# virtuoso/clap

Measured on AMD Instinct MI355X. Metric: entity updates/sec (transform hierarchy + inverse + AABB + frustum cull + visible list), higher is better.
Workload: dtype f32; 1 GPU; BASELINE configs[1]: 1000000 entities/GPU, 125000 chains x depth 8, tiles SoA layout, all dirty, fused frustum cull + ordered visible list (303309 visible); entities_per_gpu=1000000, levels=8, particles_per_gpu=0, exchange=none

## Files before the change

clap_amd/_lib.py:

```python
import ctypes as C
import os
import subprocess

_HERE = os.path.dirname(os.path.abspath(__file__))
LIB_PATH = os.environ.get("CLAPGPU_LIB") or os.path.join(_HERE, "lib", "libclapgpu.so")
CSRC = os.path.join(_HERE, "csrc")
ABI_VERSION = 46

OK = 0
ERR_NOMEM = -1
ERR_INVALID_ARGUMENTS = -2
ERR_NOT_SUPPORTED = -3
ERR_TOO_LARGE = -11
ERR_INIT_FAILED = -14
ERR_OUT_OF_BOUNDS = -26
ERR_UNKNOWN = -32

E_VISIBLE = 1 << 0
E_SKIP_CULLING = 1 << 14
E_DIRTY = 1 << 16
E_JOINT_ATTACHED = 1 << 17
E_ALIVE = 1 << 31
RAY_INVALID = 1 << 0
RAY_UNRESOLVED = 1 << 1
RAY_MOVED_TARGET = 1 << 2
SLIDE_INVALID = 1 << 0
SLIDE_UNRESOLVED = 1 << 1
SLIDE_MOVED_TARGET = 1 << 2
UPDATE_ALL_DIRTY = 1 << 0

_ERR_NAMES = {ERR_NOMEM: "NOMEM", ERR_INVALID_ARGUMENTS: "INVALID_ARGUMENTS", ERR_NOT_SUPPORTED: "NOT_SUPPORTED",
              ERR_TOO_LARGE: "TOO_LARGE", ERR_INIT_FAILED: "INITIALIZATION_FAILED",
              ERR_OUT_OF_BOUNDS: "OUT_OF_BOUNDS", ERR_UNKNOWN: "UNKNOWN_ERROR"}


class ClapGpuError(RuntimeError):
    def __init__(self, code, where, detail=""):
        self.code = code
        super().__init__(f"{where}: CERR_{_ERR_NAMES.get(code, code)} ({code}) {detail}".rstrip())


class Frustum(C.Structure):
    _fields_ = [("planes", C.c_float * 24), ("corners", C.c_float * 32)]


class BvQuery(C.Structure):
    _fields_ = [("cam_pos", C.c_float * 3), ("has_ctl", C.c_uint32), ("ctl_pos", C.c_float * 3),
                ("ctl_entity", C.c_uint32), ("result", C.c_void_p), ("inside_mask", C.c_void_p)]


EXTRA_VIEWS_MAX = 4


class Views(C.Structure):
    _fields_ = [("n", C.c_uint32), ("pad", C.c_uint32), ("frustum", Frustum * EXTRA_VIEWS_MAX),
                ("vis_mask", C.c_void_p * EXTRA_VIEWS_MAX), ("vis_row_pop", C.c_void_p * EXTRA_VIEWS_MAX),
                ("host_vis_mask", C.c_void_p * EXTRA_VIEWS_MAX)]


class Entities(C.Structure):
    _fields_ = [("n", C.c_uint32), ("n_models", C.c_uint32),
                ("pos_scale", C.c_void_p), ("rot", C.c_void_p), ("parent", C.c_void_p),
                ("model", C.c_void_p), ("model_table", C.c_void_p), ("flags", C.c_void_p),
                ("seqs", C.c_void_p), ("mx", C.c_void_p), ("inv_mx", C.c_void_p),
                ("aabb", C.c_void_p), ("center", C.c_void_p), ("vis_mask", C.c_void_p),
                ("vis_row_pop", C.c_void_p), ("n_attach", C.c_uint32), ("pad", C.c_uint32),
                ("attach", C.c_void_p), ("jt_pool", C.c_void_p), ("bind_pool", C.c_void_p),
                ("attach_local", C.c_void_p), ("bv", C.POINTER(BvQuery)), ("rebuilt_mask", C.c_void_p),
                ("views", C.POINTER(Views))]


class Particles(C.Structure):
    _fields_ = [("n", C.c_uint32), ("n_sys", C.c_uint32), ("sys", C.c_void_p), ("row_sys", C.c_void_p),
                ("pos", C.c_void_p), ("vel", C.c_void_p), ("rng_state", C.c_void_p),
                ("billboard_mx", C.c_void_p), ("respawn_mask", C.c_void_p), ("respawn_row_pop", C.c_void_p),
                ("respawn_list", C.c_void_p), ("respawn_count", C.c_void_p), ("scratch", C.c_void_p),
                ("respawn_groups", C.c_void_p)]


class AnimClock(C.Structure):
    _fields_ = [("n_chars", C.c_uint32), ("n_anims", C.c_uint32), ("anim", C.c_void_p), ("time_end", C.c_void_p),
                ("ani_time", C.c_void_p), ("speed", C.c_void_p), ("restart", C.c_void_p), ("frame_time", C.c_void_p),
                ("ended", C.c_void_p)]


class Skeleton(C.Structure):
    _fields_ = [("nr_joints", C.c_uint32), ("n_levels", C.c_uint32), ("parent", C.c_void_p), ("depth", C.c_void_p),
                ("root_pose", C.c_void_p), ("invmx", C.c_void_p), ("bind", C.c_void_p)]


class Animations(C.Structure):
    _fields_ = [("n_anims", C.c_uint32), ("n_times", C.c_uint32), ("chan_table", C.c_void_p),
                ("times", C.c_void_p), ("data", C.c_void_p), ("packed", C.c_void_p), ("packed_keys", C.c_uint32),
                ("packed_layout", C.c_uint32), ("n_data", C.c_uint32), ("pad", C.c_uint32)]


class PoseBatch(C.Structure):
    _fields_ = [("n_chars", C.c_uint32), ("skip", C.c_uint32), ("anim", C.c_void_p), ("frame_time", C.c_void_p), ("entity", C.c_void_p),
                ("entity_mx", C.c_void_p), ("trs", C.c_void_p), ("joint_transforms", C.c_void_p),
                ("joint_pos", C.c_void_p)]


class SkinBatch(C.Structure):
    _fields_ = [("n_chars", C.c_uint32), ("nr_joints", C.c_uint32), ("vert_first", C.c_void_p),
                ("vert_count", C.c_void_p), ("out_first", C.c_void_p), ("position", C.c_void_p),
                ("normal", C.c_void_p), ("joints", C.c_void_p), ("weights", C.c_void_p),
                ("joint_transforms", C.c_void_p), ("out_position", C.c_void_p), ("out_normal", C.c_void_p),
                ("out_w", C.c_void_p)]


class World(C.Structure):
    _fields_ = [("gravity", C.c_double * 3), ("linear_damping", C.c_double),
                ("linear_damping_threshold_sq", C.c_double), ("adis_linear_threshold_sq", C.c_double),
                ("adis_angular_threshold_sq", C.c_double), ("adis_time", C.c_double),
                ("adis_steps", C.c_int32), ("pad", C.c_int32)]


class Bodies(C.Structure):
    _fields_ = [("n", C.c_uint32), ("adis_average_samples", C.c_uint32), ("pos", C.c_void_p), ("quat", C.c_void_p),
                ("lvel", C.c_void_p), ("avel", C.c_void_p), ("mass", C.c_void_p), ("radius", C.c_void_p),
                ("yoffset", C.c_void_p), ("bflags", C.c_void_p), ("adis_steps_left", C.c_void_p),
                ("adis_time_left", C.c_void_p), ("body_entity", C.c_void_p),
                ("length", C.c_void_p), ("inertia", C.c_void_p), ("geom_offset_R", C.c_double * 12),
                ("aabb", C.c_void_p), ("axis", C.c_void_p), ("adis_samples", C.c_void_p), ("adis_counter", C.c_void_p),
                ("geom_records", C.c_void_p), ("facc", C.c_void_p)]


class Geoms(C.Structure):
    _fields_ = [("n", C.c_uint32), ("pad", C.c_uint32), ("pos", C.c_void_p), ("axis", C.c_void_p),
                ("radius", C.c_void_p), ("length", C.c_void_p), ("kind", C.c_void_p), ("aabb", C.c_void_p),
                ("material", C.c_void_p), ("records", C.c_void_p)]


class TrimeshDesc(C.Structure):
    _fields_ = [("n_meshes", C.c_uint32), ("n_statics", C.c_uint32), ("static_index", C.c_void_p), ("vx_first", C.c_void_p),
                ("tri_first", C.c_void_p), ("vx", C.c_void_p), ("idx", C.c_void_p), ("scale", C.c_void_p),
                ("pos", C.c_void_p), ("quat", C.c_void_p)]


POSE_SKIP_TRS, POSE_SKIP_JOINT_POS, POSE_JOINT_POS_MODEL = 1, 2, 4
BODY_DISABLED, BODY_AUTO_DISABLE, BODY_NO_GRAVITY, BODY_GYROSCOPIC, BODY_HAS_JOINT, BODY_KINEMATIC = 1, 2, 4, 8, 16, 32
GEOM_SPHERE, GEOM_CAPSULE, GEOM_BOX, GEOM_OTHER = 0, 1, 2, 3
CONTACT_DEEP = 0x80000000


def mesh_contact_scratch(static_capacity):
    return (int(static_capacity) + 63) // 64 + 1


def bodies_push_scratch_bytes(n):
    return int(lib().clapgpu_bodies_push_scratch_bytes(int(n)))


def bodies_islands_scratch_bytes(n):
    return int(lib().clapgpu_bodies_islands_scratch_bytes(int(n)))


def bodies_solve_scratch_bytes(n, rows_capacity):
    return int(lib().clapgpu_bodies_solve_scratch_bytes(int(n), int(rows_capacity)))


class Slide(C.Structure):
    _fields_ = [("n", C.c_uint32), ("body", C.c_void_p), ("velocity", C.c_void_p), ("airborne", C.c_void_p),
                ("first_frac", C.c_void_p), ("push_hit", C.c_void_p), ("flags", C.c_void_p)]


class CharactersMove(C.Structure):
    _fields_ = [("n", C.c_uint32), ("body", C.c_void_p), ("ray_off", C.c_void_p), ("motion", C.c_void_p),
                ("state", C.c_void_p), ("jump", C.c_void_p), ("jump_params", C.c_void_p), ("velocity", C.c_void_p),
                ("normal", C.c_void_p), ("airborne", C.c_void_p), ("request", C.c_void_p), ("applied", C.c_void_p),
                ("collision", C.c_void_p), ("first_frac", C.c_void_p), ("push_hit", C.c_void_p), ("flags", C.c_void_p),
                ("entity", C.c_void_p), ("yaw_quat", C.c_void_p)]


CS_START, CS_WAKING, CS_IDLE, CS_MOVING, CS_JUMP_START, CS_JUMPING, CS_FALLING, CS_NONE = 0, 1, 2, 3, 4, 5, 6, 0xff


ANIQ_MAX = 4
ANI_END_NONE, ANI_END_IDLE, ANI_END_START_MOTION, ANI_END_ANY_TO_JUMP, ANI_END_HOST = 0, 1, 2, 3, 0xff
(ANI_IDLE, ANI_START_TO_IDLE, ANI_MOTION_STOP, ANI_JUMP_TO_IDLE, ANI_FALL_TO_IDLE, ANI_MOTION, ANI_MOTION_START,
 ANI_JUMP_TO_MOTION, ANI_IDLE_TO_JUMP, ANI_MOTION_TO_JUMP, ANI_JUMP, ANI_FALL, ANI_NAMES) = range(13)
ANI_NAME_LIST = ("idle", "start_to_idle", "motion_stop", "jump_to_idle", "fall_to_idle", "motion", "motion_start",
                 "jump_to_motion", "idle_to_jump", "motion_to_jump", "jump", "fall")
ANIQ_ENDED, ANIQ_STARTED, ANIQ_ADVANCED, ANIQ_CB_IDLE, ANIQ_CB_START_MOTION, ANIQ_CB_ANY_TO_JUMP, ANIQ_HOST, ANIQ_OVERFLOW = (
    1, 2, 4, 8, 16, 32, 64, 128)
ANIQ_STATE_SHIFT = 8


class AniqEntry(C.Structure):
    _fields_ = [("animation", C.c_uint16), ("repeat", C.c_uint8), ("end", C.c_uint8), ("speed", C.c_float)]


class Aniq(C.Structure):
    _fields_ = [("n", C.c_uint32), ("n_anims", C.c_uint32), ("name_anim", C.c_void_p), ("time_end", C.c_void_p),
                ("queue", C.c_void_p), ("len", C.c_void_p), ("cur", C.c_void_p), ("cleared", C.c_void_p),
                ("ani_time", C.c_void_p), ("state", C.c_void_p), ("airborne", C.c_void_p), ("velocity", C.c_void_p),
                ("ch_motion", C.c_void_p), ("jump_params", C.c_void_p), ("mover", C.c_void_p), ("pose_anim", C.c_void_p),
                ("frame_time", C.c_void_p), ("events", C.c_void_p)]


def characters_move_scratch_bytes(n_bodies, n):
    return int(lib().clapgpu_characters_move_scratch_bytes(int(n_bodies), int(n)))


def characters_order_scratch_bytes(n, pair_capacity):
    return int(lib().clapgpu_characters_order_scratch_bytes(int(n), int(pair_capacity)))


def characters_move_ordered_scratch_bytes(n_bodies, n, pair_capacity):
    return int(lib().clapgpu_characters_move_ordered_scratch_bytes(int(n_bodies), int(n), int(pair_capacity)))


class Characters(C.Structure):
    _fields_ = [("n", C.c_uint32), ("limbo_height", C.c_float), ("entity", C.c_void_p), ("body", C.c_void_p),
                ("hist_pos", C.c_void_p), ("hist_head", C.c_void_p), ("hist_wrapped", C.c_void_p),
                ("airborne", C.c_void_p), ("moved", C.c_void_p)]


class Lights(C.Structure):
    _fields_ = [("nr_lights", C.c_uint32), ("pad", C.c_uint32), ("pos", C.c_void_p), ("color", C.c_void_p),
                ("attenuation", C.c_void_p), ("is_dir", C.c_void_p), ("active", C.c_void_p)]


class Solver(C.Structure):
    _fields_ = [("iterations", C.c_uint32), ("wide_rows", C.c_uint32), ("sor_w", C.c_double), ("cfm", C.c_double)]


class FrameDesc(C.Structure):
    _fields_ = [("entities", C.POINTER(Entities)), ("tile_row_start", C.c_void_p), ("n_tiles", C.c_uint32),
                ("level_start", C.c_void_p), ("n_levels", C.c_uint32), ("frustum", C.POINTER(Frustum)),
                ("bodies", C.POINTER(Bodies)), ("world", C.POINTER(World)), ("bp", C.c_void_p),
                ("pairs", C.c_void_p), ("pair_capacity", C.c_uint32), ("pair_total", C.c_void_p),
                ("static_pairs", C.c_void_p), ("static_pair_capacity", C.c_uint32), ("static_pair_total", C.c_void_p),
                ("body_geoms", C.POINTER(Geoms)), ("static_geoms", C.POINTER(Geoms)),
                ("contacts", C.c_void_p), ("static_contacts", C.c_void_p),
                ("contact_total", C.c_void_p), ("static_contact_total", C.c_void_p),
                ("n_body_links", C.c_uint32), ("link_body", C.c_void_p), ("link_entity", C.c_void_p),
                ("characters", C.POINTER(Characters)),
                ("lights", C.POINTER(Lights)),
                ("n_light_carriers", C.c_uint32), ("carrier_entity", C.c_void_p), ("carrier_light", C.c_void_p),
                ("carrier_offset", C.c_void_p),
                ("light_width", C.c_uint32), ("light_height", C.c_uint32), ("light_cell", C.c_uint32), ("light_tiles", C.c_void_p),
                ("view_mx", C.POINTER(C.c_float)), ("proj_mx", C.POINTER(C.c_float)),
                ("anim_clock", C.POINTER(AnimClock)), ("now_dev", C.c_void_p),
                ("skeleton", C.POINTER(Skeleton)), ("animations", C.POINTER(Animations)), ("pose", C.POINTER(PoseBatch)),
                ("skin", C.POINTER(SkinBatch)),
                ("particles", C.POINTER(Particles)),
                ("index_base", C.c_uint32), ("visible", C.c_void_p), ("visible_count", C.c_void_p), ("visible_scratch", C.c_void_p),
                ("cam_pos", C.c_float * 3), ("force_lod", C.c_void_p), ("cur_lod", C.c_void_p), ("draw_lod", C.c_void_p),
                ("flags", C.c_uint32),
                ("meshes", C.c_void_p), ("mesh_contacts", C.c_void_p), ("mesh_ref", C.c_void_p),
                ("mesh_contact_capacity", C.c_uint32), ("mesh_contact_total", C.c_void_p), ("mesh_capped", C.c_void_p),
                ("mesh_scratch", C.c_void_p),
                ("island_scratch", C.c_void_p), ("island", C.c_void_p), ("island_woken", C.c_void_p),
                ("solver", C.POINTER(Solver)), ("solve_scratch", C.c_void_p), ("solve_rows_capacity", C.c_uint32),
                ("solve_status", C.c_void_p),
                ("move", C.POINTER(CharactersMove)), ("move_dt_sec", C.c_double), ("move_scratch", C.c_void_p),
                ("aniq", C.POINTER(Aniq))]


LIGHTS_MAX = 128

STRUCTS = {
    "clapgpu_frustum": Frustum, "clapgpu_bv_query": BvQuery, "clapgpu_views": Views, "clapgpu_entities": Entities,
    "clapgpu_particles": Particles, "clapgpu_anim_clock": AnimClock, "clapgpu_skeleton": Skeleton,
    "clapgpu_animations": Animations, "clapgpu_pose_batch": PoseBatch, "clapgpu_skin_batch": SkinBatch,
    "clapgpu_world": World, "clapgpu_bodies": Bodies, "clapgpu_geoms": Geoms, "clapgpu_trimesh_desc": TrimeshDesc,
    "clapgpu_slide": Slide, "clapgpu_move": CharactersMove, "clapgpu_characters": Characters, "clapgpu_lights": Lights,
    "clapgpu_solver": Solver, "clapgpu_aniq_entry": AniqEntry, "clapgpu_aniq": Aniq, "clapgpu_frame": FrameDesc,
}


SYMBOLS = {
    "clapgpu_device_count": (C.c_int, []),
    "clapgpu_init": (C.c_int, [C.c_int]),
    "clapgpu_last_error": (C.c_char_p, []),
    "clapgpu_test_fail_after": (None, [C.c_int]),
    "clapgpu_abi_version": (C.c_uint32, []),
    "clapgpu_malloc": (C.c_int, [C.POINTER(C.c_void_p), C.c_size_t]),
    "clapgpu_free": (C.c_int, [C.c_void_p]),
    "clapgpu_host_malloc": (C.c_int, [C.POINTER(C.c_void_p), C.c_size_t]),
    "clapgpu_host_free": (C.c_int, [C.c_void_p]),
    "clapgpu_memcpy_h2d": (C.c_int, [C.c_void_p, C.c_void_p, C.c_size_t, C.c_void_p]),
    "clapgpu_memcpy_d2h": (C.c_int, [C.c_void_p, C.c_void_p, C.c_size_t, C.c_void_p]),
    "clapgpu_memset": (C.c_int, [C.c_void_p, C.c_int, C.c_size_t, C.c_void_p]),
    "clapgpu_stream_sync": (C.c_int, [C.c_void_p]),
    "clapgpu_view_matrix": (None, [C.POINTER(C.c_float), C.POINTER(C.c_float), C.POINTER(C.c_float)]),
    "clapgpu_perspective": (None, [C.c_float, C.c_float, C.c_float, C.c_float, C.c_int, C.POINTER(C.c_float)]),
    "clapgpu_frustum_calc": (None, [C.POINTER(C.c_float), C.POINTER(C.c_float), C.c_int, C.POINTER(Frustum)]),
    "clapgpu_entities_update": (C.c_int, [C.c_void_p, C.POINTER(Entities), C.POINTER(C.c_uint32), C.c_uint32,
                                          C.c_uint32, C.POINTER(Frustum)]),
    "clapgpu_entities_update_level": (C.c_int, [C.c_void_p, C.POINTER(Entities), C.c_uint32, C.c_uint32,
                                                C.c_uint32, C.POINTER(Frustum)]),
    "clapgpu_entities_update_tiles": (C.c_int, [C.c_void_p, C.POINTER(Entities), C.c_void_p, C.c_uint32,
                                                C.c_uint32, C.POINTER(Frustum)]),
    "clapgpu_entities_lod": (C.c_int, [C.c_void_p, C.POINTER(Entities), C.c_void_p, C.c_void_p, C.c_uint32,
                                       C.POINTER(C.c_float), C.c_void_p, C.c_void_p, C.c_void_p]),
    "clapgpu_entities_cull": (C.c_int, [C.c_void_p, C.POINTER(Entities), C.POINTER(Frustum)]),
    "clapgpu_visible_scratch_bytes": (C.c_size_t, [C.c_uint32]),
    "clapgpu_visible_compact": (C.c_int, [C.c_void_p, C.c_void_p, C.c_void_p, C.c_uint32, C.c_uint32, C.c_void_p,
                                          C.c_void_p, C.c_void_p]),
    "clapgpu_animation_time": (C.c_int, [C.c_void_p, C.POINTER(AnimClock), C.c_double]),
    "clapgpu_animation_time_dev": (C.c_int, [C.c_void_p, C.POINTER(AnimClock), C.c_void_p]),
    "clapgpu_animations_packed_bytes": (C.c_size_t, [C.c_uint32, C.c_uint32, C.c_uint32]),
    "clapgpu_animations_pack": (C.c_int, [C.c_void_p, C.POINTER(Animations), C.c_uint32, C.c_uint32, C.c_void_p, C.POINTER(C.c_uint32)]),
    "clapgpu_joint_pos_world": (C.c_int, [C.c_void_p, C.POINTER(Skeleton), C.POINTER(PoseBatch)]),
    "clapgpu_pose_update": (C.c_int, [C.c_void_p, C.POINTER(Skeleton), C.POINTER(Animations), C.POINTER(PoseBatch)]),
    "clapgpu_skin": (C.c_int, [C.c_void_p, C.POINTER(SkinBatch)]),
    "clapgpu_phys_step_schedule": (C.c_int, [C.POINTER(C.c_double), C.c_double]),
    "clapgpu_world_defaults": (None, [C.POINTER(World)]),
    "clapgpu_bodies_step": (C.c_int, [C.c_void_p, C.POINTER(Bodies), C.POINTER(World), C.c_double]),
    "clapgpu_phys_body_update": (C.c_int, [C.c_void_p, C.POINTER(Bodies), C.c_uint32, C.c_void_p, C.c_void_p, C.c_void_p,
                                           C.c_void_p]),
    "clapgpu_geom_offset_rotation": (None, [C.POINTER(C.c_double)]),
    "clapgpu_mass_sphere_total": (None, [C.c_double, C.c_double, C.POINTER(C.c_double)]),
    "clapgpu_mass_capsule_total": (None, [C.c_double, C.c_int, C.c_double, C.c_double, C.POINTER(C.c_double)]),
    "clapgpu_capsule_geom": (None, [C.c_float, C.c_float, C.c_float, C.c_double, C.c_double, C.POINTER(C.c_float),
                                    C.POINTER(C.c_float), C.POINTER(C.c_float), C.POINTER(C.c_int), C.POINTER(C.c_float)]),
    "clapgpu_bodies_aabb": (C.c_int, [C.c_void_p, C.POINTER(Bodies)]),
    "clapgpu_bp_create": (C.c_int, [C.POINTER(C.c_void_p), C.c_uint32, C.c_double, C.c_uint32, C.c_void_p]),
    "clapgpu_bp_create_levels": (C.c_int, [C.POINTER(C.c_void_p), C.c_uint32, C.c_double, C.c_uint32, C.c_uint32, C.c_void_p]),
    "clapgpu_bp_levels": (C.c_uint32, [C.c_void_p]),
    "clapgpu_bp_cell_slot": (C.c_uint32, [C.c_void_p, C.c_uint32, C.c_int32, C.c_int32, C.c_int32]),
    "clapgpu_bp_destroy": (None, [C.c_void_p]),
    "clapgpu_bp_collide": (C.c_int, [C.c_void_p, C.c_void_p, C.c_uint32, C.c_void_p, C.c_void_p, C.c_uint32, C.c_void_p,
                                     C.c_void_p, C.c_uint32, C.c_void_p]),
    "clapgpu_bp_status": (C.c_int, [C.c_void_p, C.c_void_p, C.POINTER(C.c_uint32)]),
    "clapgpu_bp_static_aabb": (C.c_void_p, [C.c_void_p]),
    "clapgpu_bp_statics_update": (C.c_int, [C.c_void_p, C.c_void_p, C.c_uint32, C.c_void_p]),
    "clapgpu_bp_statics_sizes": (C.c_int, [C.c_void_p, C.POINTER(C.c_uint32), C.POINTER(C.c_uint32), C.POINTER(C.c_uint32),
                                           C.POINTER(C.c_uint32), C.POINTER(C.c_double)]),
    "clapgpu_bp_statics_read": (C.c_int, [C.c_void_p, C.c_void_p, C.c_void_p, C.c_void_p, C.c_void_p, C.c_void_p, C.c_void_p]),
    "clapgpu_contacts_geoms": (C.c_int, [C.c_void_p, C.POINTER(Geoms), C.POINTER(Geoms), C.c_void_p, C.c_void_p, C.c_uint32,
                                         C.c_void_p, C.c_void_p, C.c_void_p, C.c_void_p]),
    "clapgpu_contacts_geoms_both": (C.c_int, [C.c_void_p, C.c_void_p, C.POINTER(Geoms), C.POINTER(Geoms), C.c_void_p, C.c_void_p,
                                              C.c_uint32, C.c_void_p, C.c_void_p, C.c_void_p, C.c_void_p, C.c_uint32, C.c_void_p,
                                              C.c_void_p, C.c_void_p]),
    "clapgpu_sweep_capsules": (C.c_int, [C.c_void_p, C.POINTER(Geoms), C.POINTER(Geoms), C.c_void_p, C.c_uint32, C.c_void_p,
                                         C.c_void_p, C.c_void_p, C.c_void_p, C.c_void_p, C.c_void_p, C.c_void_p]),
    "clapgpu_bodies_rotate_from_entities": (C.c_int, [C.c_void_p, C.POINTER(Bodies), C.POINTER(Entities), C.c_uint32,
                                                      C.c_uint32, C.c_void_p, C.c_void_p]),
    "clapgpu_contacts_spheres": (C.c_int, [C.c_void_p, C.POINTER(Bodies), C.c_void_p, C.c_void_p, C.c_uint32,
                                           C.c_void_p, C.c_void_p, C.c_void_p]),
    "clapgpu_contacts_sphere_box": (C.c_int, [C.c_void_p, C.POINTER(Bodies), C.c_uint32, C.c_void_p, C.c_void_p,
                                              C.c_void_p, C.c_uint32, C.c_void_p, C.c_void_p, C.c_void_p, C.c_void_p]),
    "clapgpu_shard_tile_range": (C.c_int, [C.c_void_p, C.c_uint32, C.c_uint32, C.c_uint32, C.POINTER(C.c_uint32),
                                           C.POINTER(C.c_uint32)]),
    "clapgpu_bodies_step_prebin": (C.c_int, [C.c_void_p, C.POINTER(Bodies), C.POINTER(World), C.c_double, C.c_void_p]),
    "clapgpu_bp_invalidate": (C.c_int, [C.c_void_p, C.c_void_p]),
    "clapgpu_bp_index": (C.c_int, [C.c_void_p, C.c_void_p, C.c_uint32, C.c_void_p]),
    "clapgpu_bp_index_status": (C.c_int, [C.c_void_p, C.c_void_p, C.POINTER(C.c_uint32)]),
    "clapgpu_bp_leveled_index": (C.c_int, [C.c_void_p, C.c_int]),
    "clapgpu_ray_cast": (C.c_int, [C.c_void_p, C.c_void_p, C.POINTER(Geoms), C.POINTER(Geoms), C.c_void_p, C.c_uint32,
                                   C.c_void_p, C.c_void_p, C.c_void_p, C.c_void_p, C.c_void_p, C.c_void_p]),
    "clapgpu_bodies_ground_collide": (C.c_int, [C.c_void_p, C.c_void_p, C.POINTER(Bodies), C.POINTER(Geoms), C.c_void_p,
                                                C.c_uint32, C.c_void_p, C.c_void_p, C.c_void_p, C.c_void_p, C.c_void_p,
                                                C.c_void_p, C.c_void_p, C.c_void_p, C.c_void_p]),
    "clapgpu_trimesh_create": (C.c_int, [C.c_void_p, C.POINTER(C.c_void_p), C.POINTER(TrimeshDesc)]),
    "clapgpu_trimesh_pose": (C.c_int, [C.c_void_p, C.c_void_p, C.c_void_p, C.c_void_p]),
    "clapgpu_trimesh_status": (C.c_int, [C.c_void_p, C.c_void_p, C.POINTER(C.c_uint32), C.POINTER(C.c_uint32)]),
    "clapgpu_trimesh_destroy": (None, [C.c_void_p]),
    "clapgpu_contacts_meshes": (C.c_int, [C.c_void_p, C.POINTER(Geoms), C.POINTER(Geoms), C.c_void_p, C.c_void_p, C.c_void_p,
                                          C.c_uint32, C.c_void_p, C.c_uint32, C.c_void_p, C.c_void_p, C.c_void_p, C.c_void_p,
                                          C.c_void_p]),
    "clapgpu_sweep_capsules_grid": (C.c_int, [C.c_void_p, C.c_void_p, C.POINTER(Bodies), C.POINTER(Geoms), C.c_void_p, C.c_uint32,
                                              C.c_void_p, C.c_void_p, C.c_void_p, C.c_void_p, C.c_void_p, C.c_void_p]),
    "clapgpu_characters_slide": (C.c_int, [C.c_void_p, C.c_void_p, C.POINTER(Bodies), C.POINTER(Geoms), C.c_void_p, C.c_double,
                                           C.POINTER(Slide), C.c_void_p]),
    "clapgpu_bodies_push_scratch_bytes": (C.c_size_t, [C.c_uint32]),
    "clapgpu_bodies_push": (C.c_int, [C.c_void_p, C.POINTER(Bodies), C.POINTER(World), C.c_uint32, C.c_void_p, C.c_void_p,
                                      C.c_void_p, C.c_void_p, C.c_void_p, C.c_void_p]),
    "clapgpu_characters_move_scratch_bytes": (C.c_size_t, [C.c_uint32, C.c_uint32]),
    "clapgpu_characters_move": (C.c_int, [C.c_void_p, C.c_void_p, C.POINTER(Bodies), C.POINTER(World), C.POINTER(Geoms),
                                          C.c_void_p, C.POINTER(Entities), C.c_double, C.POINTER(CharactersMove), C.c_void_p]),
    "clapgpu_characters_state": (C.c_int, [C.c_void_p, C.POINTER(Aniq), C.POINTER(CharactersMove), C.c_double, C.c_void_p]),
    "clapgpu_animation_queue_time": (C.c_int, [C.c_void_p, C.POINTER(Aniq), C.c_double, C.c_void_p]),
    "clapgpu_characters_order_scratch_bytes": (C.c_size_t, [C.c_uint32, C.c_uint32]),
    "clapgpu_characters_order": (C.c_int, [C.c_void_p, C.c_void_p, C.POINTER(Bodies), C.POINTER(World), C.c_double,
                                           C.POINTER(CharactersMove), C.c_uint32, C.c_void_p, C.c_void_p,
                                           C.POINTER(C.c_uint32), C.c_void_p]),
    "clapgpu_characters_move_ordered_scratch_bytes": (C.c_size_t, [C.c_uint32, C.c_uint32, C.c_uint32]),
    "clapgpu_characters_move_ordered": (C.c_int, [C.c_void_p, C.c_void_p, C.c_void_p, C.POINTER(Bodies), C.POINTER(World),
                                                  C.POINTER(Geoms), C.c_void_p, C.POINTER(Entities), C.c_double,
                                                  C.POINTER(CharactersMove), C.c_uint32, C.c_void_p, C.POINTER(C.c_uint32),
                                                  C.c_void_p]),
    "clapgpu_bodies_islands_scratch_bytes": (C.c_size_t, [C.c_uint32]),
    "clapgpu_bodies_islands": (C.c_int, [C.c_void_p, C.POINTER(Bodies), C.POINTER(World), C.c_double, C.c_void_p, C.c_void_p,
                                         C.c_uint32, C.c_void_p, C.c_void_p, C.c_void_p, C.c_void_p]),
    "clapgpu_solver_defaults": (None, [C.POINTER(Solver)]),
    "clapgpu_bodies_solve_scratch_bytes": (C.c_size_t, [C.c_uint32, C.c_uint32]),
    "clapgpu_bodies_solve": (C.c_int, [C.c_void_p, C.POINTER(Bodies), C.POINTER(World), C.POINTER(Solver), C.c_double, C.c_void_p,
                                       C.c_void_p, C.c_void_p, C.c_uint32, C.c_void_p,
                                       C.c_void_p, C.c_void_p, C.c_void_p, C.c_uint32,
                                       C.c_void_p, C.c_void_p, C.c_uint32, C.c_void_p,
                                       C.c_uint32, C.c_void_p, C.c_void_p, C.c_void_p, C.c_void_p, C.c_void_p,
                                       C.c_void_p, C.c_void_p]),
    "clapgpu_visible_compact_lod": (C.c_int, [C.c_void_p, C.c_void_p, C.c_uint32, C.c_void_p, C.c_void_p, C.c_void_p, C.c_void_p,
                                              C.c_void_p, C.c_void_p, C.c_void_p]),
    "clapgpu_characters_update_clock": (C.c_int, [C.c_void_p, C.c_void_p, C.c_void_p, C.c_void_p, C.c_void_p, C.c_double, C.c_void_p]),
    "clapgpu_host_malloc_mapped": (C.c_int, [C.POINTER(C.c_void_p), C.POINTER(C.c_void_p), C.c_size_t]),
    "clapgpu_entities_apply_inputs": (C.c_int, [C.c_void_p, C.c_void_p, C.c_void_p, C.c_uint32]),
    "clapgpu_entities_place": (C.c_int, [C.c_void_p, C.c_void_p, C.c_void_p, C.c_uint32, C.c_void_p]),
    "clapgpu_entities_export_rebuilt": (C.c_int, [C.c_void_p, C.c_void_p, C.c_void_p]),
    "clapgpu_entities_export_rows": (C.c_int, [C.c_void_p, C.c_void_p, C.c_void_p, C.c_void_p]),
    "clapgpu_entities_update_tiles_hostio": (C.c_int, [C.c_void_p, C.c_void_p, C.c_void_p, C.c_uint32, C.c_uint32, C.c_void_p,
                                                       C.c_void_p]),
    "clapgpu_wait_word": (C.c_int, [C.c_void_p, C.c_uint32, C.c_void_p]),
    "clapgpu_exchange_set_library": (None, [C.c_char_p]),
    "clapgpu_exchange_available": (C.c_int, []),
    "clapgpu_exchange_unique_id": (C.c_int, [C.c_void_p]),
    "clapgpu_exchange_create": (C.c_int, [C.POINTER(C.c_void_p), C.c_void_p, C.c_int, C.c_int]),
    "clapgpu_exchange_info": (C.c_int, [C.c_void_p, C.POINTER(C.c_int), C.POINTER(C.c_int), C.c_char_p]),
    "clapgpu_exchange_destroy": (None, [C.c_void_p]),
    "clapgpu_exchange_visible": (C.c_int, [C.c_void_p, C.c_void_p, C.c_void_p, C.c_uint32, C.c_void_p, C.c_void_p, C.c_void_p,
                                           C.c_void_p]),
    "clapgpu_exchange_visible_ranges": (C.c_int, [C.c_void_p, C.c_void_p, C.c_void_p, C.c_uint32, C.c_void_p, C.c_void_p, C.c_void_p,
                                                  C.c_void_p, C.c_void_p, C.c_void_p]),
    "clapgpu_visible_compact_ranges": (C.c_int, [C.c_void_p, C.c_void_p, C.c_uint32, C.c_uint32, C.c_void_p, C.c_void_p, C.c_void_p,
                                                 C.c_void_p, C.c_void_p]),
    "clapgpu_visible_expand_ranges_host": (C.c_uint32, [C.c_void_p, C.c_uint32, C.c_uint32, C.c_void_p, C.c_void_p, C.c_void_p, C.c_uint32]),
    "clapgpu_shard_bases": (C.c_int, [C.c_void_p, C.c_uint32, C.c_uint32, C.c_void_p, C.c_void_p, C.POINTER(C.c_uint32)]),
    "clapgpu_mat4_invert": (None, [C.POINTER(C.c_float), C.POINTER(C.c_float)]),
    "clapgpu_mat4_from_quat": (None, [C.POINTER(C.c_float), C.POINTER(C.c_float)]),
    "clapgpu_frame_issue": (C.c_int, [C.c_void_p, C.POINTER(FrameDesc), C.c_double, C.c_uint32]),
    "clapgpu_particles_update": (C.c_int, [C.c_void_p, C.POINTER(Particles), C.POINTER(C.c_float)]),
    "clapgpu_characters_update": (C.c_int, [C.c_void_p, C.POINTER(Characters), C.POINTER(Entities),
                                            C.POINTER(Bodies)]),
    "clapgpu_light_grid_dims": (None, [C.c_uint32, C.c_uint32, C.c_uint32, C.POINTER(C.c_uint32),
                                       C.POINTER(C.c_uint32)]),
    "clapgpu_light_grid_compute": (C.c_int, [C.c_void_p, C.POINTER(Lights), C.POINTER(C.c_float),
                                             C.POINTER(C.c_float), C.c_uint32, C.c_uint32, C.c_uint32, C.c_void_p]),
    "clapgpu_lights_from_entities": (C.c_int, [C.c_void_p, C.POINTER(Entities), C.c_uint32, C.c_uint32, C.c_void_p,
                                               C.c_void_p, C.c_void_p, C.POINTER(Lights)]),
}

_lib = None


def build(verbose=False):
    subprocess.run(["make", "-C", CSRC] + ([] if verbose else ["-s"]), check=True)


def lib():
    global _lib
    if _lib is None:
        if not os.path.exists(LIB_PATH):
            raise ClapGpuError(ERR_INIT_FAILED, "clap_amd",
                               f"{LIB_PATH} is missing: run `python -c 'import __graft_entry__ as g; g.build()'` "
                               "(there is no CPU fallback)")
        try:
            import torch
        except ImportError:
            pass
        L = C.CDLL(LIB_PATH)
        for name, (res, args) in SYMBOLS.items():
            fn = getattr(L, name)
            fn.restype = res
            fn.argtypes = args
        got = L.clapgpu_abi_version()
        if got & 0x80000000 and os.environ.get("CLAPGPU_ALLOW_EXPERIMENT") == "1":
            got &= 0x7FFFFFFF
        if got != ABI_VERSION:
            raise ClapGpuError(ERR_INIT_FAILED, "clap_amd",
                               "libclapgpu ABI version mismatch; rebuild" if not got & 0x80000000 else
                               "libclapgpu is an EXPERIMENT build (-DCLAPGPU_EXPERIMENT: kernels compiled with parts "
                               "switched off); rebuild without EXTRA=, or set CLAPGPU_ALLOW_EXPERIMENT=1 for an A/B run")
        _lib = L
    return _lib


def check(rc, where):
    if rc != OK:
        detail = lib().clapgpu_last_error()
        raise ClapGpuError(rc, where, detail.decode() if detail else "")
```

clap_amd/csrc/entities.hip:

```cpp
#include <string.h>
#include <math.h>
#include <type_traits>
#include "common.h"
#include "lm_dev.h"
#include "entities_row.h"
#include "entities_args.h"

namespace clapgpu {

template <bool CULL, bool XV = false>
__device__ __forceinline__ void process_row_fast(const EntK &e, const RowIn &in, float4 *tile, const float4 *mt,
                                                 const int lane, const uint32_t row_first, const uint32_t mode,
                                                 const lmd::FrustumK &fr, const int src, const uint32_t parent_seq_now,
                                                 float (&carry_mx)[16], uint32_t &carry_seq, const XViewsK *xv = nullptr)
{
    const uint32_t i = row_first + lane;
    const uint32_t fl = in.fl;
    const int32_t p = in.p;
    uint32_t seq = in.sq & 0xffffu, pseq = in.sq >> 16;
    float pm[16];
#pragma unroll
    for (int k = 0; k < 16; k++) pm[k] = __shfl(carry_mx[k], src);
    if (p >= 0) pseq = parent_seq_now;

    const float4 lo = mt[2 * in.mi], hi = mt[2 * in.mi + 1];
    float mx[16], inv[16], bb[6], ctr[3], local_mx[16];
    lmd::trs(local_mx, in.ps.x, in.ps.y, in.ps.z, in.ps.w, in.q.x, in.q.y, in.q.z, in.q.w);
    if (p >= 0) {
        lmd::mul(mx, pm, local_mx);
    } else {
#pragma unroll
        for (int k = 0; k < 16; k++) mx[k] = local_mx[k];
    }
    row_inverse(inv, mx);
    row_box(bb, ctr, mx, lo, hi);
    seq = (seq + 1) & 0xffffu;
#pragma unroll
    for (int k = 0; k < 16; k++) carry_mx[k] = mx[k];
    carry_seq = seq;

    const size_t e0 = row_first;
    float4 *tile_a = tile, *tile_b = tile + 256;
    float *tile_f = reinterpret_cast<float *>(tile);
    float4 va[4], vb[4];
    stage_mat4(tile_a, mx, lane);
    stage_mat4(tile_b, inv, lane);
    wave_lds_fence();
    unstage_mat4(tile_a, va, lane);
    unstage_mat4(tile_b, vb, lane);
    store_mat4_rows(e.mx + 16 * e0, va, lane, WAVE);
    store_mat4_rows(e.inv_mx + 16 * e0, vb, lane, WAVE);
    e.seqs[i] = seq | (pseq << 16);
    wave_lds_fence();
    stage_rows<6>(tile_f, bb, lane);
    wave_lds_fence();
    {
        float *ab = e.aabb + 6 * e0;
        store_stream(&reinterpret_cast<float4 *>(ab)[lane], reinterpret_cast<const float4 *>(tile_f)[lane]);
        const float2 t2 = reinterpret_cast<const float2 *>(tile_f + 4 * WAVE)[lane];
        const clapgpu_f2 v2 = { t2.x, t2.y };
        const clapgpu_f3 v3 = { ctr[0], ctr[1], ctr[2] };
        store_stream(reinterpret_cast<clapgpu_f2 *>(ab + 4 * WAVE) + lane, v2);
        store_stream(reinterpret_cast<clapgpu_f3 *>(e.center + 3 * (e0 + lane)), v3);
    }
    wave_lds_fence();
    if (!(mode & CLAPGPU_UPDATE_ALL_DIRTY) && (fl & CLAPGPU_E_DIRTY))
        e.flags[i] = fl & ~CLAPGPU_E_DIRTY;
    if (e.rebuilt_mask && lane == 0) e.rebuilt_mask[row_first >> 6] = ~0ull;
    if (CULL) {
        bool vis = (fl & CLAPGPU_E_VISIBLE) != 0;
        if (vis && !(fl & CLAPGPU_E_SKIP_CULLING))
            vis = lmd::aabb_in_frustum_fast(fr, bb);
        const uint64_t m = __ballot(vis);
        e.vis_mask[e0 >> 6] = m;
        e.vis_row_pop[e0 >> 6] = (uint8_t)__popcll(m);
        if constexpr (XV) cull_extra_views(*xv, (fl & CLAPGPU_E_VISIBLE) != 0, fl, bb, (uint32_t)(e0 >> 6), lane);
    }
}

__global__ __launch_bounds__(ENT_BLOCK)
void k_attach_prepare(EntK e)
{
    const uint32_t k = blockIdx.x * ENT_BLOCK + threadIdx.x;
    if (k >= e.n_attach) return;
    const clapgpu_attach at = e.attach[k];
    const float4 ps = e.pos_scale[at.entity], q = e.rot[at.entity];
    float local_mx[16], jt[16], bd[16], joint_mx[16], out[16];
    lmd::trs(local_mx, ps.x, ps.y, ps.z, ps.w, q.x, q.y, q.z, q.w);
    load_mat4(jt, e.jt_pool + 16 * (size_t)at.jt);
    load_mat4(bd, e.bind_pool + 16 * (size_t)at.bind);
    lmd::mul(joint_mx, jt, bd);
    lmd::mul(out, joint_mx, local_mx);
    float4 *d = reinterpret_cast<float4 *>(e.attach_local + 16 * (size_t)k);
#pragma unroll
    for (int c = 0; c < 4; c++)
        d[c] = make_float4(out[4 * c], out[4 * c + 1], out[4 * c + 2], out[4 * c + 3]);
}

template <bool CULL, class... XV>
__global__ __launch_bounds__(ENT_BLOCK)
void k_entities_level(EntK e, uint32_t first, uint32_t count, uint32_t mode, lmd::FrustumK fr, XV... xv)
{
    __shared__ float4 lds_tiles[ENT_BLOCK / WAVE][LDS_F4_PER_WAVE];
    const int lane = lane_id();
    const int wave = threadIdx.x / WAVE;
    const uint32_t wave_local0 = blockIdx.x * ENT_BLOCK + wave * WAVE;
    if (wave_local0 >= count)
        return;
    const uint32_t row_count = count - wave_local0 < WAVE ? count - wave_local0 : WAVE;
    float carry_mx[16];
    uint32_t carry_seq = 0;
    bool carry_valid = false;
    const RowIn in = load_row(e, lane, first + wave_local0, row_count);
    process_row<CULL, false, false, sizeof...(XV) != 0>(e, in, lds_tiles[wave], lane, first + wave_local0, row_count, mode, fr,
                                                        false, 0, carry_mx, carry_seq, carry_valid, nullptr, nullptr, xviews_ptr(xv...));
}

constexpr int ENT_MT_CAP = 256;
constexpr int ENT_TILE_WAVES = 1;
template <bool CULL, class... XV>
__global__ __launch_bounds__(ENT_BLOCK, ENT_TILE_WAVES)
void k_entities_tiles(lmd::FrustumK fr_arg, EntK e, const uint32_t *tile_row_start, uint32_t n_tiles, uint32_t n,
                      uint32_t mode, XV... xv)
{
#if defined(__HIP_DEVICE_COMPILE__)
    (void)fr_arg;
    typedef const __attribute__((address_space(4))) lmd::FrustumK *frustum_ptr;
    frustum_ptr frp = (frustum_ptr)__builtin_amdgcn_kernarg_segment_ptr();
#else
    typedef const lmd::FrustumK *frustum_ptr;
    frustum_ptr frp = &fr_arg;
#endif
    __shared__ float4 lds_tiles[ENT_BLOCK / WAVE][LDS_F4_PER_WAVE];
    __shared__ float4 mt_lds[2 * ENT_MT_CAP];
    const int lane = lane_id();
    const int wave = __builtin_amdgcn_readfirstlane(threadIdx.x / WAVE);
    const bool mt_cached = e.n_models <= (uint32_t)ENT_MT_CAP;
    if (mt_cached)
        for (uint32_t k = threadIdx.x; k < 2 * e.n_models; k += ENT_BLOCK) mt_lds[k] = e.model_table[k];
    __syncthreads();
    const uint32_t t = blockIdx.x * (ENT_BLOCK / WAVE) + wave;
    if (t >= n_tiles)
        return;
    const uint32_t n_rows = (n + WAVE - 1) / WAVE;
    uint32_t row = tile_row_start[t], row_end = tile_row_start[t + 1];
    if (row_end > n_rows) row_end = n_rows;
    if (row >= row_end)
        return;

    float carry_mx[16];
#pragma unroll
    for (int k = 0; k < 16; k++) carry_mx[k] = 0.f;
    uint32_t carry_seq = 0;
    bool carry_valid = false;
    bool have_prev = false;

    uint32_t row_first = row * WAVE;
    uint32_t row_count = n - row_first < WAVE ? n - row_first : WAVE;
    RowIn cur = load_row(e, lane, row_first, row_count);

    if (mt_cached && !e.bv_on) {
        asm volatile("" : : "v"(cur.ps.w), "v"(cur.q.w), "v"(cur.fl), "v"(cur.sq), "v"(cur.mi), "v"(cur.p));
        for (;;) {
            const uint32_t fl = cur.fl;
            const int32_t p = cur.p;
            const bool in_prev = have_prev && p >= 0 && (uint32_t)p >= row_first - WAVE && (uint32_t)p < row_first;
            const int src = in_prev ? (int)((uint32_t)p - (row_first - WAVE)) : lane;
            const uint32_t parent_seq_now = __shfl(carry_seq, src);
            const bool parent_ok = p < 0 || (in_prev && __shfl((int)carry_valid, src) != 0);
            const bool dirty = (mode & CLAPGPU_UPDATE_ALL_DIRTY) ? true : (fl & CLAPGPU_E_DIRTY) != 0;
            const bool rebuild = p >= 0 ? !((cur.sq >> 16) == parent_seq_now && !dirty) : dirty;
            const bool lane_ok = (fl & CLAPGPU_E_ALIVE) && rebuild && parent_ok &&
                                 !((fl & CLAPGPU_E_JOINT_ATTACHED) && e.n_attach) &&
                                 __float_as_uint(mt_lds[2 * cur.mi].w) == 0u;
            if (row_count != WAVE || __ballot(lane_ok) != ~0ull)
                break;
            const uint32_t next = row + 1;
            const bool more = next < row_end;
            const uint32_t nfirst = more ? next * WAVE : row_first;
            const uint32_t ncount = n - nfirst < WAVE ? n - nfirst : WAVE;
            const RowIn nxt = load_row(e, lane, nfirst, ncount);
            frustum_ptr frr = frp;
            asm volatile("" : "+s"(frr));
            process_row_fast<CULL, sizeof...(XV) != 0>(e, cur, lds_tiles[wave], mt_lds, lane, row_first, mode, *(const lmd::FrustumK *)frr,
                                                       src, parent_seq_now, carry_mx, carry_seq, xviews_ptr(xv...));
            carry_valid = true;
            if (!more)
                return;
            have_prev = true;
            cur = nxt;
            row = next;
            row_first = nfirst;
            row_count = ncount;
        }
    }
    for (;;) {
        const uint32_t next = row + 1;
        const bool more = next < row_end;
        const uint32_t nfirst = more ? next * WAVE : row_first;
        const uint32_t ncount = n - nfirst < WAVE ? n - nfirst : WAVE;
        const RowIn nxt = load_row(e, lane, nfirst, ncount);
        frustum_ptr frr = frp;
        asm volatile("" : "+s"(frr));
        process_row<CULL, true, false, sizeof...(XV) != 0>(e, cur, lds_tiles[wave], lane, row_first, row_count, mode, *(const lmd::FrustumK *)frr,
                                                           have_prev, row_first - WAVE, carry_mx, carry_seq, carry_valid, nullptr, nullptr,
                                                           xviews_ptr(xv...));
        if (!more)
            break;
        have_prev = true;
        cur = nxt;
        row = next;
        row_first = nfirst;
        row_count = ncount;
    }
}

template <class F> struct first_param;
template <class R, class A0, class... A> struct first_param<R (*)(A0, A...)> { using type = A0; };
static_assert(std::is_same<first_param<decltype(&k_entities_tiles<true>)>::type, lmd::FrustumK>::value &&
              std::is_same<first_param<decltype(&k_entities_tiles<false>)>::type, lmd::FrustumK>::value,
              "k_entities_tiles: the frustum must stay the first kernel argument (it is read at kernarg offset 0)");
static_assert(std::is_same<first_param<decltype(&k_entities_tiles<true, XViewsK>)>::type, lmd::FrustumK>::value, "... with further views: the same");
static_assert(alignof(lmd::FrustumK) <= 8, "kernarg offset 0 holds for any alignment the segment start guarantees");

bool make_xviews_k(const clapgpu_entities *e, bool hostio, XViewsK *out)
{
    memset(out, 0, sizeof(*out));
    const clapgpu_views *v = e->views;
    if (!v || !v->n) return true;
    if (v->n > CLAPGPU_EXTRA_VIEWS_MAX) return false;
    out->n = v->n;
    for (uint32_t k = 0; k < v->n; k++) {
        if (!v->vis_mask[k] || !v->vis_row_pop[k]) return false;
        out->mask[k] = v->vis_mask[k]; out->pop[k] = v->vis_row_pop[k];
        out->o_mask[k] = hostio ? v->host_vis_mask[k] : nullptr;
        out->fr[k] = make_frustum_k(&v->frustum[k]);
    }
    return true;
}

}

using namespace clapgpu;

static int prepare_attachments(void *stream, const EntK &k)
{
    if (!k.n_attach)
        return CLAPGPU_OK;
    hipLaunchKernelGGL(k_attach_prepare, dim3((k.n_attach + ENT_BLOCK - 1) / ENT_BLOCK), dim3(ENT_BLOCK), 0,
                       as_stream(stream), k);
    CLAPGPU_LAUNCH_CHECK("k_attach_prepare");
    return CLAPGPU_OK;
}

static int launch_level(void *stream, const EntK &k, uint32_t first, uint32_t count, uint32_t mode,
                        const clapgpu_frustum *frustum, const XViewsK &xv)
{
    const lmd::FrustumK fr = make_frustum_k(frustum);
    const dim3 grid((count + ENT_BLOCK - 1) / ENT_BLOCK), block(ENT_BLOCK);
    if (frustum && xv.n)
        hipLaunchKernelGGL((k_entities_level<true, XViewsK>), grid, block, 0, as_stream(stream), k, first, count, mode, fr, xv);
    else if (frustum)
        hipLaunchKernelGGL(k_entities_level<true>, grid, block, 0, as_stream(stream), k, first, count, mode, fr);
    else
        hipLaunchKernelGGL(k_entities_level<false>, grid, block, 0, as_stream(stream), k, first, count, mode, fr);
    CLAPGPU_LAUNCH_CHECK("k_entities_level");
    return CLAPGPU_OK;
}

extern "C" int clapgpu_entities_update_level(void *stream, const clapgpu_entities *e,
                                             uint32_t first, uint32_t count,
                                             uint32_t mode, const clapgpu_frustum *frustum)
{
    int rc = check_entities(e, frustum != nullptr);
    if (rc) return rc;
    if (first & 63u)
        return CLAPGPU_ERR_INVALID_ARGUMENTS;
    if (first > e->n || count > e->n - first)
        return CLAPGPU_ERR_OUT_OF_BOUNDS;
    if (!count)
        return CLAPGPU_OK;
    const EntK k = to_kernel_args(e);
    XViewsK xv;
    if (!make_xviews_k(e, false, &xv)) return CLAPGPU_ERR_INVALID_ARGUMENTS;
    rc = prepare_attachments(stream, k);
    if (rc) return rc;
    return launch_level(stream, k, first, count, mode, frustum, xv);
}

extern "C" int clapgpu_entities_update(void *stream, const clapgpu_entities *e,
                                       const uint32_t *level_start, uint32_t n_levels,
                                       uint32_t mode, const clapgpu_frustum *frustum)
{
    int rc = check_entities(e, frustum != nullptr);
    if (rc) return rc;
    if (!level_start || (e->n && !n_levels))
        return CLAPGPU_ERR_INVALID_ARGUMENTS;
    if (e->n == 0)
        return CLAPGPU_OK;
    if (level_start[0] != 0 || level_start[n_levels] != e->n)
        return CLAPGPU_ERR_OUT_OF_BOUNDS;
    for (uint32_t l = 0; l < n_levels; l++)
        if (level_start[l] > level_start[l + 1] || (level_start[l] & 63u))
            return CLAPGPU_ERR_INVALID_ARGUMENTS;

    const EntK k = to_kernel_args(e);
    XViewsK xv;
    if (!make_xviews_k(e, false, &xv)) return CLAPGPU_ERR_INVALID_ARGUMENTS;
    if (k.bv_result)
        CLAPGPU_HIP(hipMemsetAsync(k.bv_result, 0, sizeof(uint64_t), as_stream(stream)));
    rc = prepare_attachments(stream, k);
    if (rc) return rc;
    for (uint32_t l = 0; l < n_levels; l++) {
        const uint32_t first = level_start[l], count = level_start[l + 1] - first;
        if (!count)
            continue;
        rc = launch_level(stream, k, first, count, mode, frustum, xv);
        if (rc) return rc;
    }
    return CLAPGPU_OK;
}

extern "C" int clapgpu_entities_update_tiles(void *stream, const clapgpu_entities *e,
                                             const uint32_t *tile_row_start, uint32_t n_tiles,
                                             uint32_t mode, const clapgpu_frustum *frustum)
{
    int rc = check_entities(e, frustum != nullptr);
    if (rc) return rc;
    if (e->n == 0 || n_tiles == 0)
        return CLAPGPU_OK;
    if (!tile_row_start)
        return CLAPGPU_ERR_INVALID_ARGUMENTS;
    const lmd::FrustumK fr = make_frustum_k(frustum);
    const EntK k = to_kernel_args(e);
    XViewsK xv;
    if (!make_xviews_k(e, false, &xv)) return CLAPGPU_ERR_INVALID_ARGUMENTS;
    if (k.bv_result)
        CLAPGPU_HIP(hipMemsetAsync(k.bv_result, 0, sizeof(uint64_t), as_stream(stream)));
    rc = prepare_attachments(stream, k);
    if (rc) return rc;
    const uint32_t per_block = ENT_BLOCK / WAVE;
    const dim3 grid((n_tiles + per_block - 1) / per_block), block(ENT_BLOCK);
    if (frustum && xv.n)
        hipLaunchKernelGGL((k_entities_tiles<true, XViewsK>), grid, block, 0, as_stream(stream), fr, k, tile_row_start, n_tiles, e->n, mode, xv);
    else if (frustum)
        hipLaunchKernelGGL(k_entities_tiles<true>, grid, block, 0, as_stream(stream), fr, k, tile_row_start, n_tiles,
                           e->n, mode);
    else
        hipLaunchKernelGGL(k_entities_tiles<false>, grid, block, 0, as_stream(stream), fr, k, tile_row_start, n_tiles,
                           e->n, mode);
    CLAPGPU_LAUNCH_CHECK("k_entities_tiles");
    return CLAPGPU_OK;
}

extern "C" int clapgpu_entities_update_tiles_hostio(void *stream, const clapgpu_entities *e,
                                                    const uint32_t *tile_row_start, uint32_t n_tiles, uint32_t mode,
                                                    const clapgpu_frustum *frustum, const clapgpu_entities_hostio *io)
{
    int rc = check_entities(e, frustum != nullptr);
    if (rc) return rc;
    if (!io || !io->mx || !io->inv_mx || !io->aabb || !io->center || !io->rebuilt_mask || !io->counter || !io->done ||
        (frustum && !io->vis_mask) || (io->touched && (!io->pos_scale || !io->rot || !io->flags)) || (n_tiles && !tile_row_start))
        return CLAPGPU_ERR_INVALID_ARGUMENTS;
    if (!aligned16(io->mx) || !aligned16(io->inv_mx) || (reinterpret_cast<uintptr_t>(io->aabb) & 7u) ||
        (io->touched && (!aligned16(io->pos_scale) || !aligned16(io->rot))))
        return CLAPGPU_ERR_INVALID_ARGUMENTS;
    const lmd::FrustumK fr = make_frustum_k(frustum);
    const EntK k = to_kernel_args(e);
    if (k.bv_result)
        CLAPGPU_HIP(hipMemsetAsync(k.bv_result, 0, sizeof(uint64_t), as_stream(stream)));
    rc = prepare_attachments(stream, k);
    if (rc) return rc;
    HostIO h;
    h.pos_scale = reinterpret_cast<const float4 *>(io->pos_scale); h.rot = reinterpret_cast<const float4 *>(io->rot);
    h.flags = io->flags; h.touched = io->touched;
    h.o_mx = io->mx; h.o_inv = io->inv_mx; h.o_aabb = io->aabb; h.o_center = io->center;
    h.o_vis = io->vis_mask; h.o_rebuilt = io->rebuilt_mask; h.o_inside = io->inside_mask;
    h.counter = io->counter; h.done = io->done; h.done_value = io->done_value;
    h.keep = io->keep_mask; h.o_exported = io->exported_mask; h.stale = io->stale_mask;
    h.late_ok = io->options & CLAPGPU_HOSTIO_EXPORT_STALE_READ;
    const uint32_t tiles = e->n ? n_tiles : 0;
    XViewsK xv;
    if (!make_xviews_k(e, true, &xv)) return CLAPGPU_ERR_INVALID_ARGUMENTS;
    rc = launch_entities_tiles_host(as_stream(stream), frustum != nullptr, fr, k, h, tile_row_start, tiles, e->n, mode, xv);
    if (rc) return rc;
    return CLAPGPU_OK;
}
```

clap_amd/csrc/entities_args.h:

```cpp
#pragma once
#include "entities_row.h"

namespace clapgpu {

static inline EntK to_kernel_args(const clapgpu_entities *e)
{
    EntK k;
    k.pos_scale = reinterpret_cast<const float4 *>(e->pos_scale);
    k.rot = reinterpret_cast<const float4 *>(e->rot);
    k.parent = e->parent;
    k.model = e->model;
    k.model_table = reinterpret_cast<const float4 *>(e->model_table);
    k.flags = e->flags;
    k.seqs = e->seqs;
    k.mx = e->mx;
    k.inv_mx = e->inv_mx;
    k.aabb = e->aabb;
    k.center = e->center;
    k.vis_mask = e->vis_mask;
    k.vis_row_pop = e->vis_row_pop;
    k.n_attach = (e->attach && e->jt_pool && e->bind_pool && e->attach_local) ? e->n_attach : 0;
    k.attach = e->attach;
    k.attach_local = e->attach_local;
    k.jt_pool = e->jt_pool;
    k.bind_pool = e->bind_pool;
    k.n = e->n;
    k.n_models = e->n_models ? e->n_models : 1;
    k.bv_result = nullptr;
    k.bv_inside = nullptr;
    k.rebuilt_mask = e->rebuilt_mask;
    k.bv_has_ctl = k.bv_ctl_entity = k.bv_on = 0;
    for (int a = 0; a < 3; a++) k.bv_cam[a] = k.bv_ctl[a] = 0.f;
    if (e->bv && (e->bv->result || e->bv->inside_mask)) {
        k.bv_on = 1;
        memcpy(k.bv_cam, e->bv->cam_pos, 12);
        memcpy(k.bv_ctl, e->bv->ctl_pos, 12);
        k.bv_has_ctl = e->bv->has_ctl;
        k.bv_ctl_entity = e->bv->ctl_entity;
        k.bv_result = reinterpret_cast<unsigned long long *>(e->bv->result);
        k.bv_inside = e->bv->inside_mask;
    }
    return k;
}

static inline lmd::FrustumK make_frustum_k(const clapgpu_frustum *frustum)
{
    static_assert(sizeof(lmd::Frustum) == sizeof(clapgpu_frustum), "frustum layout");
    lmd::FrustumK k = {};
    if (!frustum)
        return k;
    memcpy(&k.f, frustum, sizeof(k.f));
    for (int ax = 0; ax < 3; ax++) {
        float lo = INFINITY, hi = -INFINITY;
        bool nan = false;
        for (int i = 0; i < 8; i++) {
            const float c = k.f.corners[i][ax];
            nan = nan || (c != c);
            lo = c < lo ? c : lo;
            hi = c > hi ? c : hi;
        }
        k.cmin[ax] = nan ? NAN : lo;
        k.cmax[ax] = nan ? NAN : hi;
    }
    k.finite = 1;
    for (int i = 0; i < 6; i++)
        for (int c = 0; c < 4; c++)
            if (!(fabsf(k.f.planes[i][c]) <= 3.402823466e+38f))
                k.finite = 0;
    return k;
}

static inline bool aligned16(const void *p) { return (reinterpret_cast<uintptr_t>(p) & 15u) == 0; }

bool make_xviews_k(const clapgpu_entities *e, bool hostio, XViewsK *out);

static inline int check_entities(const clapgpu_entities *e, bool need_mask)
{
    if (!e || !e->pos_scale || !e->rot || !e->parent || !e->model || !e->model_table || !e->flags ||
        !e->seqs || !e->mx || !e->inv_mx || !e->aabb || !e->center)
        return CLAPGPU_ERR_INVALID_ARGUMENTS;
    if (need_mask && (!e->vis_mask || !e->vis_row_pop))
        return CLAPGPU_ERR_INVALID_ARGUMENTS;
    if (!aligned16(e->pos_scale) || !aligned16(e->rot) || !aligned16(e->model_table) || !aligned16(e->mx) ||
        !aligned16(e->inv_mx) || !aligned16(e->aabb) || !aligned16(e->center))
        return CLAPGPU_ERR_INVALID_ARGUMENTS;
    return CLAPGPU_OK;
}

}
```

clap_amd/csrc/entities_row.h:

```cpp
#pragma once
#include <string.h>
#include <math.h>
#include "common.h"
#include "lm_dev.h"

namespace clapgpu {

struct EntK {
    const float4   *pos_scale;
    const float4   *rot;
    const int32_t  *parent;
    const int32_t  *model;
    const float4   *model_table;
    uint32_t       *flags;
    uint32_t       *seqs;
    float          *mx;
    float          *inv_mx;
    float          *aabb;
    float          *center;
    uint64_t       *vis_mask;
    uint8_t        *vis_row_pop;
    uint32_t        n_attach;
    const clapgpu_attach *attach;
    const float    *jt_pool;
    const float    *bind_pool;
    float          *attach_local;
    float           bv_cam[3], bv_ctl[3];
    uint32_t        bv_has_ctl, bv_ctl_entity, bv_on;
    unsigned long long *bv_result;
    uint64_t       *bv_inside;
    uint64_t       *rebuilt_mask;
    uint32_t        n, n_models;
};

struct XViewsK {
    uint32_t n, pad;
    uint64_t *mask[CLAPGPU_EXTRA_VIEWS_MAX];
    uint8_t  *pop[CLAPGPU_EXTRA_VIEWS_MAX];
    uint64_t *o_mask[CLAPGPU_EXTRA_VIEWS_MAX];
    lmd::FrustumK fr[CLAPGPU_EXTRA_VIEWS_MAX];
};

__device__ __forceinline__ const XViewsK *xviews_ptr() { return nullptr; }
__device__ __forceinline__ const XViewsK *xviews_ptr(const XViewsK &xv) { return &xv; }

__device__ __forceinline__ bool extra_view_test(const lmd::FrustumK &k, const float (&bb)[6], const float (&lo)[3], const float (&hi)[3],
                                                const bool box_finite)
{
    if (!(k.finite && box_finite))
        return lmd::aabb_in_frustum(k.f, bb);
    bool in = true;
#pragma unroll
    for (int i = 0; i < 6; i++) {
        const float x = (k.f.planes[i][0] >= 0.f) ? hi[0] : lo[0];
        const float y = (k.f.planes[i][1] >= 0.f) ? hi[1] : lo[1];
        const float z = (k.f.planes[i][2] >= 0.f) ? hi[2] : lo[2];
        float p = 0.f;
        p += x * k.f.planes[i][0];
        p += y * k.f.planes[i][1];
        p += z * k.f.planes[i][2];
        p += 1.0f * k.f.planes[i][3];
        in = in & !(p < 0.0f);
    }
#pragma unroll
    for (int ax = 0; ax < 3; ax++)
        in = in & !(k.cmin[ax] > bb[3 + ax]) & !(k.cmax[ax] < bb[ax]);
    return in;
}

__device__ __forceinline__ uint64_t cull_extra_views(const XViewsK &xv, const bool base, const uint32_t fl, const float (&bb)[6],
                                                     const uint32_t word, const int lane)
{
    uint64_t any = 0;
    const float lo[3] = { fminf(bb[0], bb[3]), fminf(bb[1], bb[4]), fminf(bb[2], bb[5]) };
    const float hi[3] = { fmaxf(bb[0], bb[3]), fmaxf(bb[1], bb[4]), fmaxf(bb[2], bb[5]) };
    bool box_finite = true;
#pragma unroll
    for (int a = 0; a < 6; a++) box_finite = box_finite && (fabsf(bb[a]) <= 3.402823466e+38f);
    const bool tested = base && !(fl & CLAPGPU_E_SKIP_CULLING);
    for (uint32_t v = 0; v < xv.n; v++) {
        const bool vis = tested ? extra_view_test(xv.fr[v], bb, lo, hi, box_finite) : base;
        const uint64_t m = __ballot(vis);
        if (lane == 0) {
            xv.mask[v][word] = m;
            xv.pop[v][word] = (uint8_t)__popcll(m);
            if (xv.o_mask[v]) xv.o_mask[v][word] = m;
        }
        any |= m;
    }
    return any;
}

constexpr int ENT_BLOCK = 256;
constexpr int LDS_F4_PER_WAVE = 512;

__device__ __forceinline__ void load_mat4(float (&m)[16], const float *src)
{
    const float4 *p = reinterpret_cast<const float4 *>(src);
#pragma unroll
    for (int c = 0; c < 4; c++) {
        float4 v = p[c];
        m[4 * c] = v.x; m[4 * c + 1] = v.y; m[4 * c + 2] = v.z; m[4 * c + 3] = v.w;
    }
}

struct RowIn {
    uint32_t fl, sq;
    int32_t  p, mi;
    float4   ps, q;
};

__device__ __forceinline__ RowIn load_row(const EntK &e, const int lane, const uint32_t row_first,
                                          const uint32_t row_count)
{
    const uint32_t i = row_first + ((uint32_t)lane < row_count ? lane : 0);
    RowIn r;
    r.fl = e.flags[i];
    r.p = e.parent[i];
    r.sq = e.seqs[i];
    r.mi = e.model[i];
    if ((uint32_t)r.p >= e.n) r.p = -1;
    if ((uint32_t)r.mi >= e.n_models) r.mi = 0;
    r.ps = e.pos_scale[i];
    r.q = e.rot[i];
    return r;
}

struct HostIO {
    const float4   *pos_scale, *rot;
    const uint32_t *flags;
    const uint64_t *touched;
    uint64_t *stale;
    uint32_t late_ok;
    float          *o_mx, *o_inv, *o_aabb, *o_center;
    uint64_t       *o_vis, *o_rebuilt, *o_inside;
    uint32_t       *counter, *done, done_value;
    const uint64_t *keep;
    uint64_t       *o_exported;
};

__device__ __forceinline__ RowIn load_row_host(const EntK &e, const HostIO &h, const int lane, const uint32_t row_first,
                                               const uint32_t row_count, const uint64_t touched)
{
    RowIn r = load_row(e, lane, row_first, row_count);
    if ((uint32_t)lane < row_count && ((touched >> lane) & 1ull)) {
        const uint32_t i = row_first + lane;
        r.fl = h.flags[i];
        r.ps = h.pos_scale[i];
        r.q = h.rot[i];
    }
    return r;
}

struct RowPre {
    float2   bb0, bb1, bb2;
    float4   lo, hi;
    float4   pm[4];
    uint32_t pseq;
};

__device__ __forceinline__ void load_row_box(const EntK &e, RowPre &r, const int lane, const uint32_t row_first, const uint32_t row_count)
{
    const uint32_t i = row_first + ((uint32_t)lane < row_count ? lane : 0);
    const float2 *b = reinterpret_cast<const float2 *>(e.aabb + 6 * (size_t)i);
    r.bb0 = b[0]; r.bb1 = b[1]; r.bb2 = b[2];
}

__device__ __forceinline__ void load_row_pre(const EntK &e, RowPre &r, const RowIn &in)
{
    r.lo = e.model_table[2 * in.mi];
    r.hi = e.model_table[2 * in.mi + 1];
    const size_t p = in.p >= 0 ? (size_t)in.p : 0;
    const float4 *m = reinterpret_cast<const float4 *>(e.mx + 16 * p);
    r.pm[0] = m[0]; r.pm[1] = m[1]; r.pm[2] = m[2]; r.pm[3] = m[3];
    r.pseq = e.seqs[p];
}

__device__ __forceinline__ int find_attach(const EntK &e, uint32_t i)
{
    uint32_t lo = 0, hi = e.n_attach;
    while (lo < hi) {
        const uint32_t mid = (lo + hi) >> 1;
        if (e.attach[mid].entity < i) lo = mid + 1; else hi = mid;
    }
    return (lo < e.n_attach && e.attach[lo].entity == i) ? (int)lo : -1;
}

__device__ __forceinline__ bool point_in_box(const float (&p)[3], const float (&bb)[6])
{
    return p[0] >= bb[0] && p[0] <= bb[3] && p[1] >= bb[1] && p[1] <= bb[4] && p[2] >= bb[2] && p[2] <= bb[5];
}

__device__ __forceinline__ void row_inverse(float (&inv)[16], const float (&mx)[16])
{
#ifdef CLAPGPU_EXP_NO_INVERT
#pragma unroll
    for (int k = 0; k < 16; k++) inv[k] = mx[k];
#else
    lmd::invert(inv, mx);
#endif
}

__device__ __forceinline__ void row_box(float (&bb)[6], float (&ctr)[3], const float (&mx)[16], const float4 &lo, const float4 &hi)
{
#ifdef CLAPGPU_EXP_NO_AABB
#pragma unroll
    for (int k = 0; k < 6; k++) bb[k] = mx[12 + k % 3] + (k < 3 ? lo.x : hi.x);
#pragma unroll
    for (int k = 0; k < 3; k++) ctr[k] = mx[12 + k];
#else
    lmd::world_aabb(bb, ctr, mx, lo.x, lo.y, lo.z, hi.x, hi.y, hi.z);
#endif
}

template <bool CULL, bool TILE, bool HOST = false, bool XV = false>
__device__ __forceinline__ void process_row(const EntK &e, const RowIn &in, float4 *tile, const int lane,
                                            const uint32_t row_first, const uint32_t row_count,
                                            const uint32_t mode, const lmd::FrustumK &fr,
                                            const bool have_prev, const uint32_t prev_first,
                                            float (&carry_mx)[16], uint32_t &carry_seq, bool &carry_valid,
                                            const HostIO *hio = nullptr, const RowPre *pre = nullptr,
                                            const XViewsK *xv = nullptr)
{
    const bool in_range = (uint32_t)lane < row_count;
    const uint32_t i = row_first + (in_range ? lane : 0);
    uint64_t host_want = ~0ull;
    bool host_filter = false;
    uint64_t stale_w = 0;
    if constexpr (HOST) {
        host_filter = hio->keep != nullptr;
        host_want = host_filter ? hio->keep[row_first >> 6] : ~0ull;
        if (hio->stale) stale_w = hio->stale[row_first >> 6];
    }

    const uint32_t fl = in.fl;
    const bool alive = in_range && (fl & CLAPGPU_E_ALIVE);
    const bool dirty = (mode & CLAPGPU_UPDATE_ALL_DIRTY) ? true : (fl & CLAPGPU_E_DIRTY) != 0;
    const int32_t p = in.p;
    uint32_t seq = in.sq & 0xffffu, pseq = in.sq >> 16;

    bool in_prev = false;
    float pm[16];
    uint32_t parent_seq_now = 0;
    bool parent_in_regs = false;
    if (TILE) {
        in_prev = have_prev && p >= 0 && (uint32_t)p >= prev_first && (uint32_t)p < prev_first + WAVE;
        const int src = in_prev ? (int)((uint32_t)p - prev_first) : lane;
#pragma unroll
        for (int k = 0; k < 16; k++) pm[k] = __shfl(carry_mx[k], src);
        parent_seq_now = __shfl(carry_seq, src);
        if constexpr (HOST) {
            const int valid = __shfl((int)carry_valid, src);
            parent_in_regs = in_prev && valid != 0;
        } else
            parent_in_regs = in_prev && (__shfl((int)carry_valid, src) != 0);
    }
    if (p >= 0 && !in_prev)
        parent_seq_now = (HOST ? pre->pseq : e.seqs[p]) & 0xffffu;

    bool rebuild = alive;
    int at = -1;
    if (alive && p >= 0 && (fl & CLAPGPU_E_JOINT_ATTACHED) && e.n_attach)
        at = find_attach(e, i);
    const bool attached = at >= 0;
    if (p >= 0) {
        if (!attached && pseq == parent_seq_now && !dirty)
            rebuild = false;
        else
            pseq = parent_seq_now;
    } else if (!dirty) {
        rebuild = false;
    }

    float mx[16], inv[16], bb[6], ctr[3];
    bool has_aabb = false;

    if (rebuild) {
        const float4 lo = HOST ? pre->lo : e.model_table[2 * in.mi];
        const float4 hi = HOST ? pre->hi : e.model_table[2 * in.mi + 1];
        float local_mx[16];
        if (attached)
            load_mat4(local_mx, e.attach_local + 16 * (size_t)at);
        else
            lmd::trs(local_mx, in.ps.x, in.ps.y, in.ps.z, in.ps.w, in.q.x, in.q.y, in.q.z, in.q.w);
        if (p >= 0) {
            if (!parent_in_regs) {
                if constexpr (HOST) {
#pragma unroll
                    for (int c = 0; c < 4; c++) {
                        pm[4 * c] = pre->pm[c].x; pm[4 * c + 1] = pre->pm[c].y; pm[4 * c + 2] = pre->pm[c].z; pm[4 * c + 3] = pre->pm[c].w;
                    }
                } else
                    load_mat4(pm, e.mx + 16 * (size_t)p);
            }
            lmd::mul(mx, pm, local_mx);
        } else {
#pragma unroll
            for (int k = 0; k < 16; k++) mx[k] = local_mx[k];
        }
        row_inverse(inv, mx);

        has_aabb = __float_as_uint(lo.w) == 0u;
        if (has_aabb)
            row_box(bb, ctr, mx, lo, hi);

        seq = (seq + 1) & 0xffffu;
        e.seqs[i] = seq | (pseq << 16);
        if (!(mode & CLAPGPU_UPDATE_ALL_DIRTY) && (fl & CLAPGPU_E_DIRTY))
            e.flags[i] = fl & ~CLAPGPU_E_DIRTY;
    }

    if (TILE) {
#pragma unroll
        for (int k = 0; k < 16; k++) carry_mx[k] = mx[k];
        carry_seq = seq;
        carry_valid = rebuild;
    }

    const uint64_t rebuilt_mask = __ballot(rebuild);
    if (e.rebuilt_mask && lane == 0) e.rebuilt_mask[row_first >> 6] = rebuilt_mask;
    const uint64_t aabb_mask = __ballot(rebuild && has_aabb);
    const uint64_t full = row_count == WAVE ? ~0ull : ((1ull << row_count) - 1ull);
    const size_t e0 = row_first;
    float4 *tile_a = tile, *tile_b = tile + 256;
    float *tile_f = reinterpret_cast<float *>(tile);

    if (rebuilt_mask == full) {
        float4 va[4], vb[4];
        stage_mat4(tile_a, mx, lane);
        stage_mat4(tile_b, inv, lane);
        wave_lds_fence();
        unstage_mat4(tile_a, va, lane);
        unstage_mat4(tile_b, vb, lane);
        store_mat4_rows(e.mx + 16 * e0, va, lane, (int)row_count);
        store_mat4_rows(e.inv_mx + 16 * e0, vb, lane, (int)row_count);
        wave_lds_fence();
    } else if (rebuild) {
        float4 *dm = reinterpret_cast<float4 *>(e.mx + 16 * (size_t)i);
        float4 *di = reinterpret_cast<float4 *>(e.inv_mx + 16 * (size_t)i);
#pragma unroll
        for (int c = 0; c < 4; c++) {
            dm[c] = make_float4(mx[4 * c], mx[4 * c + 1], mx[4 * c + 2], mx[4 * c + 3]);
            di[c] = make_float4(inv[4 * c], inv[4 * c + 1], inv[4 * c + 2], inv[4 * c + 3]);
        }
    }
    if (aabb_mask == full) {
        stage_rows<6>(tile_f, bb, lane);
        stage_rows<3>(tile_f + 6 * WAVE, ctr, lane);
        wave_lds_fence();
        store_rows<6>(tile_f, e.aabb + 6 * e0, lane, (int)row_count);
        store_rows<3>(tile_f + 6 * WAVE, e.center + 3 * e0, lane, (int)row_count);
        wave_lds_fence();
    } else if (rebuild && has_aabb) {
#pragma unroll
        for (int k = 0; k < 6; k++) e.aabb[6 * (size_t)i + k] = bb[k];
#pragma unroll
        for (int k = 0; k < 3; k++) e.center[3 * (size_t)i + k] = ctr[k];
    }

    const bool want_bv = e.bv_on != 0;
    if (CULL || want_bv) {
        if (in_range && !(rebuild && has_aabb)) {
            if constexpr (HOST) {
                bb[0] = pre->bb0.x; bb[1] = pre->bb0.y; bb[2] = pre->bb1.x; bb[3] = pre->bb1.y; bb[4] = pre->bb2.x; bb[5] = pre->bb2.y;
            } else {
#pragma unroll
                for (int k = 0; k < 6; k++) bb[k] = e.aabb[6 * (size_t)i + k];
            }
        }
    }
    if (want_bv) {
        bool inside = in_range && (fl & CLAPGPU_E_ALIVE) && point_in_box(e.bv_cam, bb);
        if (!inside && e.bv_has_ctl)
            inside = in_range && (fl & CLAPGPU_E_ALIVE) && point_in_box(e.bv_ctl, bb);
        if (inside && e.bv_has_ctl && i == e.bv_ctl_entity)
            inside = false;
        const uint64_t inside_mask = __ballot(inside);
        if (e.bv_inside && lane == 0) e.bv_inside[e0 >> 6] = inside_mask;
        if constexpr (HOST) {
            if (hio->o_inside && lane == 0) hio->o_inside[e0 >> 6] = inside_mask;
            host_want |= inside_mask;
        }
        if (inside_mask) {
            unsigned long long key = 0;
            if (inside) {
                const float4 lo = e.model_table[2 * in.mi], hi = e.model_table[2 * in.mi + 1];
                const float X = fabsf(hi.x - lo.x) * in.ps.w, Y = fabsf(hi.y - lo.y) * in.ps.w,
                            Z = fabsf(hi.z - lo.z) * in.ps.w;
                const float vol = X * Y * Z;
                key = ((unsigned long long)__float_as_uint(vol) << 32) | (0xFFFFFFFFu - i);
            }
#pragma unroll
            for (int off = 32; off > 0; off >>= 1) {
                const unsigned long long o = __shfl_xor(key, off);
                key = o > key ? o : key;
            }
            if (lane == 0 && key && e.bv_result)
                atomicMax(e.bv_result, key);
        }
    }
    if (CULL) {
        bool vis = in_range && (fl & CLAPGPU_E_ALIVE) && (fl & CLAPGPU_E_VISIBLE);
        if (vis && !(fl & CLAPGPU_E_SKIP_CULLING))
            vis = lmd::aabb_in_frustum_fast(fr, bb);
        const uint64_t m = __ballot(vis);
        if (lane == 0) {
            e.vis_mask[e0 >> 6] = m;
            e.vis_row_pop[e0 >> 6] = (uint8_t)__popcll(m);
            if constexpr (HOST) hio->o_vis[e0 >> 6] = m;
        }
        if constexpr (HOST) host_want |= m;
        if constexpr (XV) {
            const uint64_t mx_any = cull_extra_views(*xv, in_range && (fl & CLAPGPU_E_ALIVE) && (fl & CLAPGPU_E_VISIBLE), fl, bb,
                                                     (uint32_t)(e0 >> 6), lane);
            if constexpr (HOST) host_want |= mx_any;
        }
    } else {
        if constexpr (HOST) host_want = ~0ull;
    }

    if constexpr (HOST) {
        const uint64_t exported = host_filter ? (rebuilt_mask & host_want) : rebuilt_mask;
        if (rebuild && ((exported >> lane) & 1ull)) {
            float4 *hm = reinterpret_cast<float4 *>(hio->o_mx + 16 * (size_t)i);
            float4 *hi = reinterpret_cast<float4 *>(hio->o_inv + 16 * (size_t)i);
#pragma unroll
            for (int c = 0; c < 4; c++) {
                hm[c] = make_float4(mx[4 * c], mx[4 * c + 1], mx[4 * c + 2], mx[4 * c + 3]);
                hi[c] = make_float4(inv[4 * c], inv[4 * c + 1], inv[4 * c + 2], inv[4 * c + 3]);
            }
            if (has_aabb) {
                float2 *hb = reinterpret_cast<float2 *>(hio->o_aabb + 6 * (size_t)i);
                hb[0] = make_float2(bb[0], bb[1]); hb[1] = make_float2(bb[2], bb[3]); hb[2] = make_float2(bb[4], bb[5]);
                float *hc = hio->o_center + 3 * (size_t)i;
                hc[0] = ctr[0]; hc[1] = ctr[1]; hc[2] = ctr[2];
            }
        }
        const uint64_t late = hio->late_ok ? stale_w & host_want & ~rebuilt_mask & __ballot(alive) : 0ull;
        if ((late >> lane) & 1ull) {
            const float4 *sm = reinterpret_cast<const float4 *>(e.mx + 16 * (size_t)i);
            const float4 *si = reinterpret_cast<const float4 *>(e.inv_mx + 16 * (size_t)i);
            float4 *hm = reinterpret_cast<float4 *>(hio->o_mx + 16 * (size_t)i);
            float4 *hi = reinterpret_cast<float4 *>(hio->o_inv + 16 * (size_t)i);
#pragma unroll
            for (int c = 0; c < 4; c++) { hm[c] = sm[c]; hi[c] = si[c]; }
            const float2 *sb = reinterpret_cast<const float2 *>(e.aabb + 6 * (size_t)i);
            float2 *hb = reinterpret_cast<float2 *>(hio->o_aabb + 6 * (size_t)i);
            hb[0] = sb[0]; hb[1] = sb[1]; hb[2] = sb[2];
            const float *sc = e.center + 3 * (size_t)i;
            float *hc = hio->o_center + 3 * (size_t)i;
            hc[0] = sc[0]; hc[1] = sc[1]; hc[2] = sc[2];
        }
        if (lane == 0) {
            hio->o_rebuilt[row_first >> 6] = rebuilt_mask;
            if (hio->o_exported) hio->o_exported[row_first >> 6] = exported | late;
            if (hio->stale) {
                const uint64_t ns = (stale_w | rebuilt_mask) & ~(exported | late);
                if (ns != stale_w) hio->stale[row_first >> 6] = ns;
            }
        }
    }
}

__device__ __forceinline__ void raise_done_when_last(uint32_t *counter, uint32_t *done, const uint32_t done_value)
{
    __threadfence_system();
    __syncthreads();
    if (threadIdx.x == 0) {
        const uint32_t arrived = atomicAdd(counter, 1u);
        if (arrived == gridDim.x - 1) {
            *counter = 0;
            __threadfence_system();
            __hip_atomic_store(done, done_value, __ATOMIC_RELEASE, __HIP_MEMORY_SCOPE_SYSTEM);
        }
    }
}

int launch_entities_tiles_host(hipStream_t stream, bool cull, const lmd::FrustumK &fr, const EntK &e, const HostIO &h,
                               const uint32_t *tile_row_start, uint32_t n_tiles, uint32_t n, uint32_t mode, const XViewsK &xv);

}
```

clap_amd/entities.py:

```python
import ctypes as C

import numpy as np
import torch

from . import _lib
from . import synth
from ._dev import device_array, ptr as _ptr, stream as _stream, upload


def view_calc_frustum(cam):
    L = _lib.lib()
    f32p = C.POINTER(C.c_float)
    pos = np.ascontiguousarray(cam["cam_pos"], np.float32)
    quat = np.ascontiguousarray(cam["cam_quat"], np.float32)
    view = np.zeros(16, np.float32)
    proj = np.zeros(16, np.float32)
    L.clapgpu_view_matrix(pos.ctypes.data_as(f32p), quat.ctypes.data_as(f32p), view.ctypes.data_as(f32p))
    fov, aspect, near, far = (float(v) for v in cam["persp"])
    z01 = int(cam["ndc_z_zero_one"][0])
    L.clapgpu_perspective(fov, aspect, near, far, z01, proj.ctypes.data_as(f32p))
    fr = _lib.Frustum()
    L.clapgpu_frustum_calc(view.ctypes.data_as(f32p), proj.ctypes.data_as(f32p), z01, C.byref(fr))
    return fr, view, proj


def frustum_arrays(fr):
    return (np.ctypeslib.as_array(fr.planes).reshape(6, 4).copy(),
            np.ctypeslib.as_array(fr.corners).reshape(8, 4).copy())


class EntityBatch:

    IN_KEYS = ("pos_scale", "rot", "parent", "model", "flags", "seqs")

    def __init__(self, scene, device="cuda:0"):
        self.device = torch.device(device)
        dev = self.device
        self.n = int(scene["n"])
        self.n_real = int(scene.get("n_real", self.n))
        self.tiled = "tile_row_start" in scene
        if self.tiled:
            trs = np.ascontiguousarray(scene["tile_row_start"], np.uint32)
            if int(trs[-1]) * 64 != self.n:
                raise ValueError("tile_row_start does not cover the scene")
            self.n_tiles = len(trs) - 1
            self.tile_row_start = upload(trs, np.uint32, dev)
            self.level_start, self.n_levels = None, 0
        else:
            ls = np.asarray(scene["level_start"], np.uint32)
            if np.any(ls[:-1] % 64):
                raise ValueError("level starts must be multiples of 64: use synth.pad_levels()")
            self.level_start = np.ascontiguousarray(ls)
            self.n_levels = len(ls) - 1
            self._ls_ptr = self.level_start.ctypes.data_as(C.POINTER(C.c_uint32))
        for k in self.IN_KEYS:
            setattr(self, k, upload(scene[k], scene[k].dtype, dev))
        self.model_table = upload(synth.model_table(scene), np.float32, dev)
        n = self.n
        self.mx = device_array((n, 16), torch.float32, dev)
        self.inv_mx = device_array((n, 16), torch.float32, dev)
        self.aabb = device_array((n, 6), torch.float32, dev)
        self.center = device_array((n, 3), torch.float32, dev)
        self.vis_mask = device_array(((n + 63) // 64 or 1,), torch.int64, dev)
        n_rows = (n + 63) // 64
        self.vis_row_pop = device_array(((n_rows + 15) // 16 * 16 or 16,), torch.uint8, dev)
        self.visible = device_array((max(n, 1),), torch.int32, dev)
        self.visible_count = device_array((1,), torch.int32, dev)
        nscratch = _lib.lib().clapgpu_visible_scratch_bytes(n)
        self.scratch = device_array((nscratch // 4 or 1,), torch.int32, dev)
        self._desc = _lib.Entities(
            n=n, n_models=self.model_table.shape[0],
            pos_scale=self.pos_scale.data_ptr(), rot=self.rot.data_ptr(), parent=self.parent.data_ptr(),
            model=self.model.data_ptr(), model_table=self.model_table.data_ptr(), flags=self.flags.data_ptr(),
            seqs=self.seqs.data_ptr(), mx=self.mx.data_ptr(), inv_mx=self.inv_mx.data_ptr(),
            aabb=self.aabb.data_ptr(), center=self.center.data_ptr(), vis_mask=self.vis_mask.data_ptr(),
            vis_row_pop=self.vis_row_pop.data_ptr())

    def use_vis_buffers(self, vis_mask, vis_row_pop):
        self.vis_mask, self.vis_row_pop = vis_mask, vis_row_pop
        self._desc.vis_mask = vis_mask.data_ptr()
        self._desc.vis_row_pop = vis_row_pop.data_ptr()

    def set_views(self, frusta):
        dev = self.device
        n_rows = (self.n + 63) // 64
        self._views = _lib.Views()
        self._views.n = len(frusta)
        self.view_masks, self.view_row_pops = [], []
        for v, fr in enumerate(frusta[:_lib.EXTRA_VIEWS_MAX]):
            C.memmove(C.byref(self._views.frustum[v]), C.byref(fr), C.sizeof(_lib.Frustum))
            m = device_array((n_rows or 1,), torch.int64, dev)
            p = device_array(((n_rows + 15) // 16 * 16 or 16,), torch.uint8, dev)
            self.view_masks.append(m); self.view_row_pops.append(p)
            self._views.vis_mask[v] = m.data_ptr(); self._views.vis_row_pop[v] = p.data_ptr()
        self._desc.views = C.pointer(self._views) if frusta else None

    def compact_view(self, v, index_base=0):
        rc = _lib.lib().clapgpu_visible_compact(_stream(), _ptr(self.view_masks[v]), _ptr(self.view_row_pops[v]), self.n,
                                                index_base, _ptr(self.visible), _ptr(self.visible_count), _ptr(self.scratch))
        _lib.check(rc, "clapgpu_visible_compact")

    def set_attachments(self, attach, jt_pool, bind_pool):
        a = np.ascontiguousarray(attach)
        assert np.all(np.diff(a["entity"].astype(np.int64)) > 0), "attach table must be sorted by entity"
        self._attach = upload(a.view(np.uint8), np.uint8, self.device, (-1, 16))
        self._jt_pool = jt_pool if torch.is_tensor(jt_pool) else upload(jt_pool, np.float32, self.device)
        self._bind_pool = upload(bind_pool, np.float32, self.device)
        idx = upload(a["entity"], np.int64, self.device)
        self.flags[idx] |= np.int32(_lib.E_JOINT_ATTACHED)
        self._desc.n_attach = a.shape[0]
        self._desc.attach = self._attach.data_ptr()
        self._desc.jt_pool = self._jt_pool.data_ptr()
        self._desc.bind_pool = self._bind_pool.data_ptr()
        self._attach_local = device_array((a.shape[0], 16), torch.float32, self.device)
        self._desc.attach_local = self._attach_local.data_ptr()

    def set_bv_query(self, cam_pos, ctl_pos=None, ctl_entity=0):
        self.bv_result = device_array(1, torch.int64, self.device)
        q = _lib.BvQuery()
        q.cam_pos[:] = [float(v) for v in cam_pos]
        q.has_ctl = 0 if ctl_pos is None else 1
        q.ctl_pos[:] = [0.0, 0.0, 0.0] if ctl_pos is None else [float(v) for v in ctl_pos]
        q.ctl_entity = int(ctl_entity)
        q.result = self.bv_result.data_ptr()
        self._bv = q
        self._desc.bv = C.pointer(q)

    def camera_bv(self):
        key = int(self.bv_result.item()) & 0xFFFFFFFFFFFFFFFF
        if key == 0:
            return -1, 0.0
        return 0xFFFFFFFF - (key & 0xFFFFFFFF), float(np.asarray([key >> 32], np.uint32).view(np.float32)[0])

    def mq_update(self, frustum=None, all_dirty=False):
        mode = _lib.UPDATE_ALL_DIRTY if all_dirty else 0
        fr = C.byref(frustum) if frustum is not None else None
        if self.tiled:
            rc = _lib.lib().clapgpu_entities_update_tiles(_stream(), C.byref(self._desc), _ptr(self.tile_row_start),
                                                          self.n_tiles, mode, fr)
            _lib.check(rc, "clapgpu_entities_update_tiles")
        else:
            rc = _lib.lib().clapgpu_entities_update(_stream(), C.byref(self._desc), self._ls_ptr, self.n_levels,
                                                    mode, fr)
            _lib.check(rc, "clapgpu_entities_update")

    def update_level(self, level, frustum=None, all_dirty=False):
        first = int(self.level_start[level])
        count = int(self.level_start[level + 1]) - first
        mode = _lib.UPDATE_ALL_DIRTY if all_dirty else 0
        rc = _lib.lib().clapgpu_entities_update_level(_stream(), C.byref(self._desc), first, count, mode,
                                                      C.byref(frustum) if frustum is not None else None)
        _lib.check(rc, "clapgpu_entities_update_level")

    def cull(self, frustum):
        rc = _lib.lib().clapgpu_entities_cull(_stream(), C.byref(self._desc), C.byref(frustum))
        _lib.check(rc, "clapgpu_entities_cull")

    def compact_visible(self, index_base=0, two_pass=False):
        rc = _lib.lib().clapgpu_visible_compact(_stream(), _ptr(self.vis_mask),
                                                None if two_pass else _ptr(self.vis_row_pop), self.n, index_base,
                                                _ptr(self.visible), _ptr(self.visible_count), _ptr(self.scratch))
        _lib.check(rc, "clapgpu_visible_compact")

    def alloc_lod(self):
        if not hasattr(self, "cur_lod"):
            self.cur_lod = device_array(max(self.n, 1), torch.int32, self.device)
            self.draw_lod = device_array(max(self.n, 1), torch.int32, self.device)
            self.force_lod = None

    def select_lod(self, cam_pos, force_lod=None):
        self.alloc_lod()
        if force_lod is not None:
            self.force_lod = upload(force_lod, np.int32, self.device)
        cp = (C.c_float * 3)(*[float(v) for v in cam_pos])
        rc = _lib.lib().clapgpu_entities_lod(_stream(), C.byref(self._desc), _ptr(self.visible),
                                             _ptr(self.visible_count), 0, cp, _ptr(self.force_lod),
                                             _ptr(self.cur_lod), _ptr(self.draw_lod))
        _lib.check(rc, "clapgpu_entities_lod")

    def compact_visible_lod(self, cam_pos, force_lod=None, index_base=0):
        self.alloc_lod()
        if force_lod is not None:
            self.force_lod = upload(force_lod, np.int32, self.device)
        cp = (C.c_float * 3)(*[float(v) for v in cam_pos])
        rc = _lib.lib().clapgpu_visible_compact_lod(_stream(), C.byref(self._desc), index_base, cp, _ptr(self.force_lod),
                                                    _ptr(self.cur_lod), _ptr(self.visible), _ptr(self.visible_count),
                                                    _ptr(self.draw_lod), _ptr(self.scratch))
        _lib.check(rc, "clapgpu_visible_compact_lod")

    def view_entity_in_frustum(self, idx):
        w = int(self.vis_mask[idx >> 6].item()) & 0xFFFFFFFFFFFFFFFF
        return bool((w >> (idx & 63)) & 1)

    def set_transforms(self, idx, pos_scale, rot):
        idx_t = upload(idx, np.int64, self.device)
        self.pos_scale[idx_t] = upload(pos_scale, np.float32, self.device)
        self.rot[idx_t] = upload(rot, np.float32, self.device)
        self.flags[idx_t] |= np.int32(_lib.E_DIRTY)

    def download(self):
        torch.cuda.synchronize(self.device)
        cnt = int(self.visible_count.item())
        return dict(mx=self.mx.cpu().numpy(), inv_mx=self.inv_mx.cpu().numpy(), aabb=self.aabb.cpu().numpy(),
                    center=self.center.cpu().numpy(), flags=self.flags.cpu().numpy().view(np.uint32),
                    seqs=self.seqs.cpu().numpy().view(np.uint32),
                    vis_mask=self.vis_mask.cpu().numpy().view(np.uint64),
                    visible=self.visible[:cnt].cpu().numpy().view(np.uint32), visible_count=cnt)

    def algorithmic_bytes(self):
        par = self.parent.cpu().numpy()
        real = (self.flags.cpu().numpy().view(np.uint32) & np.uint32(_lib.E_ALIVE)) != 0
        children = int(np.count_nonzero((par >= 0) & real))
        roots = int(np.count_nonzero((par < 0) & real))
        return 276 * children + 212 * roots
```

clap_amd/shard.py:

```python
import numpy as np
import torch
import torch.distributed as dist

from ._dev import device_array, upload


def shard_tile_ranges(rows_per_tile, world):
    import ctypes as C
    from . import _lib
    rows = np.asarray(rows_per_tile, np.int64)
    trs = np.ascontiguousarray(np.concatenate([[0], np.cumsum(rows)]), np.uint32)
    out = []
    for r in range(world):
        t0, t1 = C.c_uint32(), C.c_uint32()
        _lib.check(_lib.lib().clapgpu_shard_tile_range(trs.ctypes.data, len(rows), r, world, C.byref(t0), C.byref(t1)),
                   "clapgpu_shard_tile_range")
        out.append((t0.value, t1.value))
    return out


def shard_bases(tile_row_start, world):
    import ctypes as C
    from . import _lib
    trs = np.ascontiguousarray(tile_row_start, np.uint32)
    base, n_pad, cap = np.zeros(world, np.uint32), np.zeros(world, np.uint32), C.c_uint32()
    _lib.check(_lib.lib().clapgpu_shard_bases(trs.ctypes.data, len(trs) - 1, world, base.ctypes.data, n_pad.ctypes.data,
                                              C.byref(cap)), "clapgpu_shard_bases")
    return base, n_pad, int(cap.value)


def expand_ranges_host(gathered_mask, world, cap_pad, base, n_pad):
    from . import _lib
    g = np.ascontiguousarray(gathered_mask).view(np.uint64)
    base, n_pad = np.ascontiguousarray(base, np.uint32), np.ascontiguousarray(n_pad, np.uint32)
    L = _lib.lib()
    n = L.clapgpu_visible_expand_ranges_host(g.ctypes.data, world, cap_pad, base.ctypes.data, n_pad.ctypes.data, None, 0)
    out = np.zeros(max(int(n), 1), np.uint32)
    got = L.clapgpu_visible_expand_ranges_host(g.ctypes.data, world, cap_pad, base.ctypes.data, n_pad.ctypes.data, out.ctypes.data, int(n))
    assert got == n
    return out[:n]


def allgather_visible(visible, count, world, counts_buf=None, gather_buf=None, pad_to=4096, group=None):
    if counts_buf is None:
        counts_buf = device_array(world, count.dtype, count.device, fill=None)
    dist.all_gather_into_tensor(counts_buf, count, group=group)
    cap = int(counts_buf.max().item())
    cap = max((cap + pad_to - 1) // pad_to * pad_to, pad_to)
    cap = min(cap, visible.shape[0])
    if gather_buf is None or gather_buf.numel() < world * cap:
        gather_buf = device_array(world * cap, visible.dtype, visible.device, fill=None)
    out = gather_buf[:world * cap]
    dist.all_gather_into_tensor(out, visible[:cap].contiguous(), group=group)
    return counts_buf, out.view(world, cap)


def allgather_visible_mask(vis_mask, world, out=None, group=None):
    n_words = vis_mask.numel()
    if out is None:
        out = device_array(world * n_words, vis_mask.dtype, vis_mask.device, fill=None)
    dist.all_gather_into_tensor(out[:world * n_words], vis_mask, group=group)
    return out


def concat_visible(counts, gathered):
    c = counts.tolist()
    return torch.cat([gathered[r, :c[r]] for r in range(len(c))])


class VisibleExchange:

    def __init__(self, batch, rank, world, device, route="rccl", share=None):
        import ctypes as C
        from . import _lib
        self._C, self._lib = C, _lib
        self.batch, self.rank, self.world, self.device = batch, rank, world, device
        self.n_pad = batch.n
        sizes = device_array(world, torch.int64, device)
        sizes[rank] = self.n_pad
        dist.all_reduce(sizes)
        self.n_pad_all = np.ascontiguousarray(sizes.cpu().numpy(), np.uint32)
        self.base = np.ascontiguousarray(np.concatenate([[0], np.cumsum(self.n_pad_all.astype(np.int64))[:-1]]), np.uint32)
        self.cap_pad = max(64, int(self.n_pad_all.max()))
        if int(self.n_pad_all.astype(np.int64).sum()) > 0xffffffff:
            raise ValueError("the scene's global ids do not fit 32 bits")
        n_words = self.cap_pad // 64
        own = batch.vis_mask.numel()

        def mask_buf():
            return device_array(n_words, batch.vis_mask.dtype, device)
        self.masks = [mask_buf(), mask_buf()]
        self.masks[0][:own].copy_(batch.vis_mask)
        pop = batch.vis_row_pop
        self.pops = [pop, device_array(pop.shape, pop.dtype, pop.device)]
        self.g_mask = [device_array(world * n_words, torch.int64, device) for _ in range(2)]
        self.g_vis = [device_array(world * self.cap_pad, torch.int32, device) for _ in range(2)]
        self.g_cnt = [device_array(1, torch.int32, device) for _ in range(2)]
        nscratch = _lib.lib().clapgpu_visible_scratch_bytes(world * self.cap_pad)
        self.g_scratch = device_array(nscratch // 4 + 4, torch.int32, device)
        self.comm = torch.cuda.Stream(device=device)
        self.ev_upd = [torch.cuda.Event() for _ in range(2)]
        self.ev_comm = [torch.cuda.Event() for _ in range(2)]
        self.frame = 0
        self.direct = None
        self.owns_direct = True
        if share is not None:
            self.direct, self.owns_direct = share.direct, False
        elif route == "rccl":
            import os
            import sys
            L = _lib.lib()
            path = os.path.join(os.path.dirname(torch.__file__), "lib", "librccl.so")
            if os.path.exists(path):
                L.clapgpu_exchange_set_library(path.encode())
            can = upload([int(L.clapgpu_exchange_available())], np.int32, device)
            dist.all_reduce(can, op=dist.ReduceOp.MIN)
            if int(can.item()) == 1:
                try:
                    self.direct = self._create_exchange(rank, world, device)
                except Exception as exc:
                    print(f"[clap_amd.shard] clapgpu_exchange unavailable ({exc}); using torch.distributed", file=sys.stderr)
                ok = upload([1 if self.direct is not None else 0], np.int32, device)
                dist.all_reduce(ok, op=dist.ReduceOp.MIN)
                if int(ok.item()) == 0 and self.direct is not None:
                    L.clapgpu_exchange_destroy(self.direct)
                    self.direct = None
            elif rank == 0:
                print("[clap_amd.shard] RCCL cannot be opened on every rank; using torch.distributed", file=sys.stderr)

    def _create_exchange(self, rank, world, device):
        C, _lib = self._C, self._lib
        L = _lib.lib()
        uid = (C.c_uint8 * 128)()
        if rank == 0 and L.clapgpu_exchange_unique_id(uid) != 0:
            uid = (C.c_uint8 * 128)()
        t = upload(np.frombuffer(bytearray(bytes(uid)), np.uint8), np.uint8, device)
        dist.broadcast(t, src=0)
        raw = (C.c_uint8 * 128).from_buffer_copy(bytes(t.cpu().numpy().tobytes()))
        if not any(raw):
            raise RuntimeError("rank 0 could not create an RCCL unique id: " + (L.clapgpu_last_error() or b"").decode())
        x = C.c_void_p()
        _lib.check(L.clapgpu_exchange_create(C.byref(x), raw, rank, world), "clapgpu_exchange_create")
        return x

    @property
    def route(self):
        return "ncclAllGather via clapgpu_exchange_visible (C)" if self.direct is not None else "torch.distributed all_gather"

    def begin(self):
        b = self.frame & 1
        torch.cuda.current_stream().wait_event(self.ev_comm[b])
        self.batch.use_vis_buffers(self.masks[b], self.pops[b])
        return b

    def submit(self):
        C, _lib = self._C, self._lib
        b = self.frame & 1
        self.frame += 1
        main = torch.cuda.current_stream()
        self.ev_upd[b].record(main)
        with torch.cuda.stream(self.comm):
            self.comm.wait_event(self.ev_upd[b])
            if self.direct is not None:
                rc = _lib.lib().clapgpu_exchange_visible_ranges(C.c_void_p(self.comm.cuda_stream), self.direct,
                                                                self.masks[b].data_ptr(), self.cap_pad, self.base.ctypes.data,
                                                                self.n_pad_all.ctypes.data, self.g_mask[b].data_ptr(),
                                                                self.g_vis[b].data_ptr(), self.g_cnt[b].data_ptr(),
                                                                self.g_scratch.data_ptr())
                _lib.check(rc, "clapgpu_exchange_visible_ranges")
            else:
                allgather_visible_mask(self.masks[b], self.world, self.g_mask[b])
                rc = _lib.lib().clapgpu_visible_compact_ranges(C.c_void_p(self.comm.cuda_stream), self.g_mask[b].data_ptr(),
                                                               self.world, self.cap_pad, self.base.ctypes.data,
                                                               self.n_pad_all.ctypes.data, self.g_vis[b].data_ptr(),
                                                               self.g_cnt[b].data_ptr(), self.g_scratch.data_ptr())
                _lib.check(rc, "clapgpu_visible_compact_ranges(global)")
            self.ev_comm[b].record(self.comm)

    def last(self):
        b = (self.frame - 1) & 1
        return self.g_cnt[b], self.g_vis[b]

    def proof(self):
        import ctypes as C
        L = self._lib.lib()
        ranks, me, bus = C.c_int(0), C.c_int(-1), C.create_string_buffer(32)
        if self.direct is not None and L.clapgpu_exchange_info(self.direct, C.byref(ranks), C.byref(me), bus) == 0:
            info = dict(rccl_ranks=int(ranks.value), comm_rank=int(me.value), device=bus.value.decode())
        else:
            props = torch.cuda.get_device_properties(self.device)
            busid = getattr(props, "pci_bus_id", None)
            info = dict(rccl_ranks=dist.get_world_size(), comm_rank=dist.get_rank(),
                        device=f"{getattr(props, 'pci_domain_id', 0):04x}:{busid:02x}:{getattr(props, 'pci_device_id', 0):02x}.0"
                        if busid is not None else f"uuid:{getattr(props, 'uuid', self.device)}")
        every = [None] * self.world
        dist.all_gather_object(every, info)
        return dict(rccl_ranks=min(e["rccl_ranks"] for e in every),
                    comm_rank_ok=all(e["comm_rank"] == r for r, e in enumerate(every)),
                    devices=[e["device"] for e in every])

    def destroy(self):
        if self.direct is not None and self.owns_direct:
            self._lib.lib().clapgpu_exchange_destroy(self.direct)
        self.direct = None
```

include/clapgpu.h:

```cpp
#ifndef CLAPGPU_H
#define CLAPGPU_H

#include <stddef.h>
#include <stdint.h>

#ifdef __cplusplus
extern "C" {
#endif

#define CLAPGPU_OK                      0
#define CLAPGPU_ERR_NOMEM              -1
#define CLAPGPU_ERR_INVALID_ARGUMENTS  -2
#define CLAPGPU_ERR_NOT_SUPPORTED      -3
#define CLAPGPU_ERR_TOO_LARGE         -11
#define CLAPGPU_ERR_INIT_FAILED       -14
#define CLAPGPU_ERR_OUT_OF_BOUNDS     -26
#define CLAPGPU_ERR_UNKNOWN           -32

#define CLAPGPU_E_VISIBLE       (1u << 0)
#define CLAPGPU_E_SKIP_CULLING  (1u << 14)
#define CLAPGPU_E_DIRTY         (1u << 16)
#define CLAPGPU_E_JOINT_ATTACHED (1u << 17)
#define CLAPGPU_E_ALIVE         (1u << 31)

int clapgpu_device_count(void);
int clapgpu_init(int device);
const char *clapgpu_last_error(void);
void clapgpu_test_fail_after(int launches);
#define CLAPGPU_ABI_VERSION 46u
uint32_t clapgpu_abi_version(void);

int clapgpu_malloc(void **dev, size_t bytes);
int clapgpu_free(void *dev);
int clapgpu_host_malloc(void **host, size_t bytes);
int clapgpu_host_malloc_mapped(void **host, void **dev_alias, size_t bytes);
int clapgpu_host_free(void *host);
int clapgpu_memcpy_h2d(void *dev, const void *host, size_t bytes, void *stream);
int clapgpu_memcpy_d2h(void *host, const void *dev, size_t bytes, void *stream);
int clapgpu_memset(void *dev, int value, size_t bytes, void *stream);
int clapgpu_stream_sync(void *stream);


typedef struct clapgpu_frustum {
    float planes[6][4];
    float corners[8][4];
} clapgpu_frustum;

void clapgpu_view_matrix(const float pos[3], const float quat[4], float view_mx[16]);
void clapgpu_mat4_invert(const float m[16], float out[16]);
void clapgpu_mat4_from_quat(const float quat_xyzw[4], float out[16]);
void clapgpu_perspective(float fov, float aspect, float near_plane, float far_plane,
                         int ndc_z_zero_one, float proj_mx[16]);
void clapgpu_frustum_calc(const float view_mx[16], const float proj_mx[16],
                          int ndc_z_zero_one, clapgpu_frustum *out);

typedef struct clapgpu_attach {
    uint32_t entity, jt, bind, pad;
} clapgpu_attach;

typedef struct clapgpu_bv_query {
    float     cam_pos[3];
    uint32_t  has_ctl;
    float     ctl_pos[3];
    uint32_t  ctl_entity;
    uint64_t *result;
    uint64_t *inside_mask;
} clapgpu_bv_query;

#define CLAPGPU_EXTRA_VIEWS_MAX 4
typedef struct clapgpu_views {
    uint32_t        n, pad;
    clapgpu_frustum frustum[CLAPGPU_EXTRA_VIEWS_MAX];
    uint64_t       *vis_mask[CLAPGPU_EXTRA_VIEWS_MAX];
    uint8_t        *vis_row_pop[CLAPGPU_EXTRA_VIEWS_MAX];
    uint64_t       *host_vis_mask[CLAPGPU_EXTRA_VIEWS_MAX];
} clapgpu_views;

typedef struct clapgpu_entities {
    uint32_t        n;
    uint32_t        n_models;
    const float    *pos_scale;
    const float    *rot;
    const int32_t  *parent;
    const int32_t  *model;
    const float    *model_table;
    uint32_t       *flags;
    uint32_t       *seqs;
    float          *mx;
    float          *inv_mx;
    float          *aabb;
    float          *center;
    uint64_t       *vis_mask;
    uint8_t        *vis_row_pop;
    uint32_t        n_attach;
    uint32_t        pad;
    const clapgpu_attach *attach;
    const float    *jt_pool;
    const float    *bind_pool;
    float          *attach_local;
    const clapgpu_bv_query *bv;
    uint64_t       *rebuilt_mask;
    const clapgpu_views *views;
} clapgpu_entities;

#define CLAPGPU_UPDATE_ALL_DIRTY  (1u << 0)

int clapgpu_entities_update(void *stream, const clapgpu_entities *e,
                            const uint32_t *level_start, uint32_t n_levels,
                            uint32_t mode, const clapgpu_frustum *frustum);

int clapgpu_entities_update_level(void *stream, const clapgpu_entities *e,
                                  uint32_t first, uint32_t count,
                                  uint32_t mode, const clapgpu_frustum *frustum);

int clapgpu_entities_update_tiles(void *stream, const clapgpu_entities *e,
                                  const uint32_t *tile_row_start, uint32_t n_tiles,
                                  uint32_t mode, const clapgpu_frustum *frustum);

int clapgpu_entities_cull(void *stream, const clapgpu_entities *e, const clapgpu_frustum *frustum);

typedef struct clapgpu_entity_input {
    uint32_t slot, flags;
    float    pos_scale[4], rot[4];
} clapgpu_entity_input;
typedef struct clapgpu_entities_export {
    float    *mx, *inv_mx, *aabb, *center;
    uint64_t *vis_mask, *rebuilt_mask, *inside_mask;
    uint32_t *counter;
    uint32_t *done;
    uint32_t  done_value, pad;
    uint64_t *stale_mask;
} clapgpu_entities_export;
int clapgpu_entities_apply_inputs(void *stream, const clapgpu_entities *e, const clapgpu_entity_input *list, uint32_t n_list);
int clapgpu_entities_export_rebuilt(void *stream, const clapgpu_entities *e, const clapgpu_entities_export *x);
typedef struct clapgpu_entity_place { uint32_t slot; int32_t parent, model; uint32_t flags; } clapgpu_entity_place;
#define CLAPGPU_PLACE_ZERO_BOX    1u
#define CLAPGPU_PLACE_CLEAR_STALE 2u
int clapgpu_entities_place(void *stream, const clapgpu_entities *e, const clapgpu_entity_place *list, uint32_t n_list,
                           uint64_t *stale_mask);
int clapgpu_entities_export_rows(void *stream, const clapgpu_entities *e, const clapgpu_entities_export *x,
                                 const uint64_t *select_mask);

#define CLAPGPU_HOSTIO_EXPORT_STALE_READ 1u
typedef struct clapgpu_entities_hostio {
    const float    *pos_scale, *rot;
    const uint32_t *flags;
    const uint64_t *touched;
    float    *mx, *inv_mx, *aabb, *center;
    uint64_t *vis_mask, *rebuilt_mask, *inside_mask;
    uint32_t *counter;
    uint32_t *done;
    uint32_t  done_value, options;
    const uint64_t *keep_mask;
    uint64_t       *exported_mask;
    uint64_t       *stale_mask;
} clapgpu_entities_hostio;
int clapgpu_entities_update_tiles_hostio(void *stream, const clapgpu_entities *e, const uint32_t *tile_row_start,
                                         uint32_t n_tiles, uint32_t mode, const clapgpu_frustum *frustum,
                                         const clapgpu_entities_hostio *io);
int clapgpu_wait_word(const volatile uint32_t *word, uint32_t value, void *stream);

size_t clapgpu_visible_scratch_bytes(uint32_t n);
int clapgpu_visible_compact(void *stream, const uint64_t *vis_mask, const uint8_t *vis_row_pop,
                            uint32_t n, uint32_t index_base, uint32_t *visible, uint32_t *count,
                            void *scratch);

int clapgpu_entities_lod(void *stream, const clapgpu_entities *e, const uint32_t *visible,
                         const uint32_t *count, uint32_t index_base, const float cam_pos[3],
                         const int32_t *force_lod, int32_t *cur_lod, int32_t *draw_lod);
int clapgpu_visible_compact_lod(void *stream, const clapgpu_entities *e, uint32_t index_base, const float cam_pos[3],
                                const int32_t *force_lod, int32_t *cur_lod, uint32_t *visible, uint32_t *count,
                                int32_t *draw_lod, void *scratch);


int clapgpu_shard_tile_range(const uint32_t *tile_row_start, uint32_t n_tiles, uint32_t rank, uint32_t world,
                             uint32_t *first_tile, uint32_t *end_tile);

#define CLAPGPU_EXCHANGE_ID_BYTES 128
typedef struct clapgpu_exchange clapgpu_exchange;
void clapgpu_exchange_set_library(const char *path);
int  clapgpu_exchange_available(void);
int  clapgpu_exchange_unique_id(uint8_t id[CLAPGPU_EXCHANGE_ID_BYTES]);
int  clapgpu_exchange_create(clapgpu_exchange **out, const uint8_t id[CLAPGPU_EXCHANGE_ID_BYTES], int rank, int world);
int  clapgpu_exchange_info(const clapgpu_exchange *x, int *comm_ranks, int *comm_rank, char pci_bus_id[32]);
void clapgpu_exchange_destroy(clapgpu_exchange *x);
int  clapgpu_exchange_visible(void *stream, clapgpu_exchange *x, const uint64_t *vis_mask, uint32_t n_pad,
                              uint64_t *gathered_mask, uint32_t *visible, uint32_t *visible_count, void *scratch);
int  clapgpu_exchange_visible_ranges(void *stream, clapgpu_exchange *x, const uint64_t *vis_mask, uint32_t cap_pad,
                                     const uint32_t *base, const uint32_t *n_pad, uint64_t *gathered_mask,
                                     uint32_t *visible, uint32_t *visible_count, void *scratch);
int  clapgpu_visible_compact_ranges(void *stream, const uint64_t *gathered_mask, uint32_t n_ranges, uint32_t cap_pad,
                                    const uint32_t *base, const uint32_t *n_pad, uint32_t *visible, uint32_t *count, void *scratch);
uint32_t clapgpu_visible_expand_ranges_host(const uint64_t *gathered_mask, uint32_t n_ranges, uint32_t cap_pad,
                                            const uint32_t *base, const uint32_t *n_pad, uint32_t *visible, uint32_t capacity);
int  clapgpu_shard_bases(const uint32_t *tile_row_start, uint32_t n_tiles, uint32_t world, uint32_t *base, uint32_t *n_pad,
                         uint32_t *cap_pad);


#define CLAPGPU_PART_DIST_LIN     0
#define CLAPGPU_PART_DIST_SQRT    1
#define CLAPGPU_PART_DIST_CBRT    2
#define CLAPGPU_PART_DIST_POW075  3

typedef struct clapgpu_particle_system {
    float    center[3];
    uint32_t dist;
    double   radius, min_radius, radius_squared, velocity;
    uint32_t first, count;
    uint32_t pad[2];
} clapgpu_particle_system;

#define CLAPGPU_RESPAWN_GROUP_WORDS 132
typedef struct clapgpu_particles {
    uint32_t  n;
    uint32_t  n_sys;
    const clapgpu_particle_system *sys;
    const uint32_t *row_sys;
    float    *pos;
    float    *vel;
    uint64_t *rng_state;
    float    *billboard_mx;
    uint64_t *respawn_mask;
    uint8_t  *respawn_row_pop;
    uint32_t *respawn_list;
    uint32_t *respawn_count;
    void     *scratch;
    uint32_t *respawn_groups;
} clapgpu_particles;

int clapgpu_particles_update(void *stream, const clapgpu_particles *p, const float view_mx[16]);


typedef struct clapgpu_skeleton {
    uint32_t        nr_joints;
    uint32_t        n_levels;
    const int32_t  *parent;
    const int32_t  *depth;
    const float    *root_pose;
    const float    *invmx;
    const float    *bind;
} clapgpu_skeleton;

typedef struct clapgpu_animations {
    uint32_t        n_anims;
    uint32_t        n_times;
    const uint32_t *chan_table;
    const float    *times;
    const float    *data;
    const void     *packed;
    uint32_t        packed_keys, packed_layout;
    uint32_t        n_data, pad;
} clapgpu_animations;

size_t clapgpu_animations_packed_bytes(uint32_t n_anims, uint32_t max_keys, uint32_t nr_joints);
int    clapgpu_animations_pack(void *stream, const clapgpu_animations *an, uint32_t nr_joints, uint32_t max_keys, void *packed,
                               uint32_t *packed_layout);

#define CLAPGPU_POSE_SKIP_TRS        (1u << 0)
#define CLAPGPU_POSE_SKIP_JOINT_POS  (1u << 1)
#define CLAPGPU_POSE_JOINT_POS_MODEL (1u << 2)
typedef struct clapgpu_pose_batch {
    uint32_t        n_chars;
    uint32_t        skip;
    const uint32_t *anim;
    const float    *frame_time;
    const uint32_t *entity;
    const float    *entity_mx;
    float          *trs;
    float          *joint_transforms;
    float          *joint_pos;
} clapgpu_pose_batch;

typedef struct clapgpu_anim_clock {
    uint32_t        n_chars;
    uint32_t        n_anims;
    const uint32_t *anim;
    const float    *time_end;
    double         *ani_time;
    const float    *speed;
    const uint8_t  *restart;
    float          *frame_time;
    uint8_t        *ended;
} clapgpu_anim_clock;
int clapgpu_animation_time(void *stream, const clapgpu_anim_clock *clk, double now);
int clapgpu_animation_time_dev(void *stream, const clapgpu_anim_clock *clk, const double *now_dev);

int clapgpu_pose_update(void *stream, const clapgpu_skeleton *sk, const clapgpu_animations *an,
                        const clapgpu_pose_batch *pb);
int clapgpu_joint_pos_world(void *stream, const clapgpu_skeleton *sk, const clapgpu_pose_batch *pb);


typedef struct clapgpu_skin_batch {
    uint32_t        n_chars;
    uint32_t        nr_joints;
    const uint32_t *vert_first;
    const uint32_t *vert_count;
    const uint32_t *out_first;
    const float    *position;
    const float    *normal;
    const uint8_t  *joints;
    const float    *weights;
    const float    *joint_transforms;
    float          *out_position;
    float          *out_normal;
    float          *out_w;
} clapgpu_skin_batch;

int clapgpu_skin(void *stream, const clapgpu_skin_batch *b);


#define CLAPGPU_BODY_DISABLED      (1u << 0)
#define CLAPGPU_BODY_AUTO_DISABLE  (1u << 1)
#define CLAPGPU_BODY_NO_GRAVITY    (1u << 2)

typedef struct clapgpu_world {
    double  gravity[3];
    double  linear_damping;
    double  linear_damping_threshold_sq;
    double  adis_linear_threshold_sq;
    double  adis_angular_threshold_sq;
    double  adis_time;
    int32_t adis_steps;
    int32_t pad;
} clapgpu_world;

#define CLAPGPU_BODY_GYROSCOPIC    (1u << 3)
#define CLAPGPU_BODY_HAS_JOINT     (1u << 4)
#define CLAPGPU_BODY_KINEMATIC     (1u << 5)
#define CLAPGPU_GEOM_SPHERE  0
#define CLAPGPU_GEOM_CAPSULE 1
#define CLAPGPU_GEOM_BOX     2
#define CLAPGPU_GEOM_OTHER   3

typedef struct clapgpu_bodies {
    uint32_t        n;
    uint32_t        adis_average_samples;
    double         *pos;
    double         *quat;
    double         *lvel;
    double         *avel;
    const double   *mass;
    const double   *radius;
    const double   *yoffset;
    uint32_t       *bflags;
    int32_t        *adis_steps_left;
    double         *adis_time_left;
    const int32_t  *body_entity;
    const double   *length;
    const double   *inertia;
    double          geom_offset_R[12];
    double         *aabb;
    double         *axis;
    double         *adis_samples;
    uint32_t       *adis_counter;
    double         *geom_records;
    double         *facc;
} clapgpu_bodies;

void clapgpu_geom_offset_rotation(double R[12]);
void clapgpu_mass_sphere_total(double total_mass, double radius, double I[3]);
void clapgpu_mass_capsule_total(double total_mass, int direction, double radius, double length, double I[3]);
void clapgpu_capsule_geom(float X, float Y, float Z, double geom_radius, double geom_offset,
                          float *radius, float *length, float *yoffset, int *direction, float *ray_off);
int clapgpu_bodies_aabb(void *stream, const clapgpu_bodies *b);

int  clapgpu_phys_step_schedule(double *time_acc, double dt);
void clapgpu_world_defaults(clapgpu_world *w);

int clapgpu_bodies_step(void *stream, const clapgpu_bodies *b, const clapgpu_world *w, double h);
struct clapgpu_bp;
int clapgpu_bodies_step_prebin(void *stream, const clapgpu_bodies *b, const clapgpu_world *w, double h, struct clapgpu_bp *bp);
int clapgpu_bp_invalidate(void *stream, struct clapgpu_bp *bp);

int clapgpu_phys_body_update(void *stream, const clapgpu_bodies *b, uint32_t n_entities, float *pos_scale,
                             float *rot, uint32_t *entity_flags, uint8_t *moving);

int clapgpu_bodies_rotate_from_entities(void *stream, const clapgpu_bodies *b, const clapgpu_entities *e,
                                        uint32_t mode, uint32_t n_links, const uint32_t *link_body,
                                        const uint32_t *link_entity);

#define CLAPGPU_CONTACT_BOUNCE   0x004
#define CLAPGPU_CONTACT_SOFT_ERP 0x008
#define CLAPGPU_CONTACT_SOFT_CFM 0x010
typedef struct clapgpu_contact {
    double   pos[3], normal[3], depth;
    double   mu, bounce, bounce_vel, soft_erp, soft_cfm;
    uint32_t mode;
    uint32_t nc;
} clapgpu_contact;
int clapgpu_contacts_spheres(void *stream, const clapgpu_bodies *b, const uint32_t *pairs,
                             const uint32_t *pair_total, uint32_t capacity, const double *material,
                             clapgpu_contact *contacts, uint32_t *contact_total);
int clapgpu_contacts_sphere_box(void *stream, const clapgpu_bodies *b, uint32_t n_static,
                                const double *static_aabb, const uint32_t *pairs, const uint32_t *pair_total,
                                uint32_t capacity, const double *material, const double *static_material,
                                clapgpu_contact *contacts, uint32_t *contact_total);

#define CLAPGPU_BP_LEVELS_MAX 16
typedef struct clapgpu_bp clapgpu_bp;
typedef struct clapgpu_trimesh clapgpu_trimesh;
int  clapgpu_bp_create(clapgpu_bp **out, uint32_t n_max, double cell, uint32_t n_static, const double *static_aabb_host);
int      clapgpu_bp_create_levels(clapgpu_bp **out, uint32_t n_max, double cell, uint32_t levels,
                                  uint32_t n_static, const double *static_aabb_host);
uint32_t clapgpu_bp_levels(const clapgpu_bp *bp);
uint32_t clapgpu_bp_cell_slot(const clapgpu_bp *bp, uint32_t level, int32_t cx, int32_t cy, int32_t cz);
void clapgpu_bp_destroy(clapgpu_bp *bp);
int  clapgpu_bp_collide(void *stream, clapgpu_bp *bp, uint32_t n, const double *aabb,
                        uint32_t *pairs, uint32_t capacity, uint32_t *pair_total,
                        uint32_t *static_pairs, uint32_t static_capacity, uint32_t *static_pair_total);
int  clapgpu_bp_status(void *stream, clapgpu_bp *bp, uint32_t *status);
const double *clapgpu_bp_static_aabb(const clapgpu_bp *bp);

int clapgpu_bp_statics_update(void *stream, clapgpu_bp *bp, uint32_t n_static, const double *static_aabb);
int clapgpu_bp_statics_sizes(const clapgpu_bp *bp, uint32_t *buckets, uint32_t *n_entries, uint32_t *n_large,
                             uint32_t large_start[CLAPGPU_BP_LEVELS_MAX + 1], double bounds[6]);
int clapgpu_bp_statics_read(void *stream, const clapgpu_bp *bp, uint32_t *start, uint32_t *entries, uint32_t *large,
                            double *entry_boxes, double *large_boxes);

typedef struct clapgpu_geoms {
    uint32_t        n, pad;
    const double   *pos;
    const double   *axis;
    const double   *radius, *length;
    const uint8_t  *kind;
    const double   *aabb;
    const double   *material;
    const double   *records;
} clapgpu_geoms;
#define CLAPGPU_CONTACT_DEEP 0x80000000u
typedef struct clapgpu_contact2 {
    double   pos[3], normal[3], depth;
    double   mu, bounce, bounce_vel, soft_erp, soft_cfm;
    uint32_t mode;
    uint32_t nc;
    double   pos2[3], normal2[3], depth2;
} clapgpu_contact2;
int clapgpu_contacts_geoms(void *stream, const clapgpu_geoms *A, const clapgpu_geoms *B, const uint32_t *pairs,
                           const uint32_t *pair_total, uint32_t capacity, clapgpu_contact2 *contacts,
                           uint32_t *contact_total, uint32_t *body_flags_a, uint32_t *body_flags_b);
int clapgpu_contacts_geoms_both(void *stream, clapgpu_bp *bp, const clapgpu_geoms *bodies, const clapgpu_geoms *statics,
                                const uint32_t *pairs, const uint32_t *pair_total, uint32_t capacity,
                                clapgpu_contact2 *contacts, uint32_t *contact_total,
                                const uint32_t *static_pairs, const uint32_t *static_pair_total, uint32_t static_capacity,
                                clapgpu_contact2 *static_contacts, uint32_t *static_contact_total, uint32_t *body_flags);

int clapgpu_sweep_capsules(void *stream, const clapgpu_geoms *A, const clapgpu_geoms *B, const clapgpu_trimesh *meshes,
                           uint32_t n_sweeps, const uint32_t *sweep_body, const float *delta, const uint32_t *cand_first,
                           const uint32_t *cand, float *frac, float *normal, int32_t *hit);

#define CLAPGPU_RAY_INVALID      1u
#define CLAPGPU_RAY_UNRESOLVED   2u
#define CLAPGPU_RAY_MOVED_TARGET 4u
int clapgpu_bp_index(void *stream, clapgpu_bp *bp, uint32_t n, const double *aabb);
int clapgpu_bp_index_status(void *stream, clapgpu_bp *bp, uint32_t *status);
int clapgpu_bp_leveled_index(clapgpu_bp *bp, int on);
int clapgpu_ray_cast(void *stream, clapgpu_bp *bp, const clapgpu_geoms *bodies, const clapgpu_geoms *statics,
                     const clapgpu_trimesh *meshes, uint32_t n_rays, const double *ray, const int32_t *skip,
                     double *dist, int32_t *hit, double *contact, uint32_t *flags);
int clapgpu_bodies_ground_collide(void *stream, clapgpu_bp *bp, const clapgpu_bodies *b, const clapgpu_geoms *statics,
                                  const clapgpu_trimesh *meshes, uint32_t n, const uint32_t *body, const double *ray_off,
                                  const uint8_t *grounded, uint8_t *grounded_out, float *normal, double *dist, int32_t *hit,
                                  uint32_t *flags, uint32_t *scratch);

typedef struct clapgpu_trimesh_desc {
    uint32_t        n_meshes, n_statics;
    const uint32_t *static_index;
    const uint32_t *vx_first, *tri_first;
    const float    *vx;
    const uint16_t *idx;
    const float    *scale;
    const double   *pos;
    const float    *quat;
} clapgpu_trimesh_desc;
int  clapgpu_trimesh_create(void *stream, clapgpu_trimesh **out, const clapgpu_trimesh_desc *d);
int  clapgpu_trimesh_pose(void *stream, clapgpu_trimesh *mesh, const double *pos, const float *quat);
int  clapgpu_trimesh_status(void *stream, const clapgpu_trimesh *mesh, uint32_t *depth, uint32_t *n_tris);
void clapgpu_trimesh_destroy(clapgpu_trimesh *mesh);

#define CLAPGPU_MESH_CONTACT_SCRATCH(static_capacity) (((static_capacity) + 63u) / 64u + 1u)
int  clapgpu_contacts_meshes(void *stream, const clapgpu_geoms *bodies, const clapgpu_geoms *statics,
                             const clapgpu_trimesh *meshes, const uint32_t *static_pairs, const uint32_t *static_pair_total,
                             uint32_t static_capacity, uint32_t *scratch, uint32_t capacity, clapgpu_contact2 *contacts,
                             uint32_t *mesh_ref, uint32_t *contact_total, uint32_t *capped_pairs, uint32_t *body_flags);

#define CLAPGPU_SLIDE_INVALID      1u
#define CLAPGPU_SLIDE_UNRESOLVED   2u
#define CLAPGPU_SLIDE_MOVED_TARGET 4u
int  clapgpu_sweep_capsules_grid(void *stream, clapgpu_bp *bp, const clapgpu_bodies *b, const clapgpu_geoms *statics,
                                 const clapgpu_trimesh *meshes, uint32_t n_sweeps, const uint32_t *sweep_body,
                                 const float *delta, float *frac, float *normal, int32_t *hit, uint32_t *flags);

typedef struct clapgpu_slide {
    uint32_t        n;
    const uint32_t *body;
    float          *velocity;
    const uint8_t  *airborne;
    float          *first_frac;
    int32_t        *push_hit;
    uint32_t       *flags;
} clapgpu_slide;
int  clapgpu_characters_slide(void *stream, clapgpu_bp *bp, const clapgpu_bodies *b, const clapgpu_geoms *statics,
                              const clapgpu_trimesh *meshes, double dt_sec, const clapgpu_slide *s, uint32_t *scratch);

size_t clapgpu_bodies_push_scratch_bytes(uint32_t n);
int  clapgpu_bodies_push(void *stream, const clapgpu_bodies *b, const clapgpu_world *w, uint32_t n, const uint32_t *pusher,
                         const float *velocity, const int32_t *push_hit, const uint32_t *flags, uint32_t *pushed,
                         void *scratch);

size_t clapgpu_bodies_islands_scratch_bytes(uint32_t n);
int  clapgpu_bodies_islands(void *stream, const clapgpu_bodies *b, const clapgpu_world *w, double h,
                            const uint32_t *pairs, const uint32_t *pair_total, uint32_t capacity,
                            const clapgpu_contact2 *contacts, void *scratch, uint32_t *island, uint32_t *woken_total);

#define CLAPGPU_SOLVE_WIDE_WORKGROUPS 1024u
typedef struct clapgpu_solver { uint32_t iterations; uint32_t wide_rows; double sor_w; double cfm; } clapgpu_solver;
void   clapgpu_solver_defaults(clapgpu_solver *s);
size_t clapgpu_bodies_solve_scratch_bytes(uint32_t n, uint32_t rows_capacity);
int    clapgpu_bodies_solve(void *stream, const clapgpu_bodies *b, const clapgpu_world *w, const clapgpu_solver *s, double h,
                            const uint32_t *island,
                            const uint32_t *static_pairs, const uint32_t *static_pair_total, uint32_t static_capacity,
                            const clapgpu_contact2 *static_contacts,
                            const clapgpu_contact2 *mesh_contacts, const uint32_t *mesh_ref,
                            const uint32_t *mesh_contact_total, uint32_t mesh_capacity,
                            const uint32_t *pairs, const uint32_t *pair_total, uint32_t capacity,
                            const clapgpu_contact2 *contacts,
                            uint32_t rows_capacity, void *scratch,
                            double *row_lambda, uint64_t *row_key,
                            uint32_t *rows_total, uint32_t *status,
                            uint32_t *row_level, uint32_t *wide_total);


#define CLAPGPU_POS_HISTORY_MAX 8

typedef struct clapgpu_characters {
    uint32_t        n;
    float           limbo_height;
    const uint32_t *entity;
    const int32_t  *body;
    float          *hist_pos;
    uint32_t       *hist_head;
    uint8_t        *hist_wrapped;
    const uint8_t  *airborne;
    uint8_t        *moved;
} clapgpu_characters;

int clapgpu_characters_update(void *stream, const clapgpu_characters *c, const clapgpu_entities *e,
                              const clapgpu_bodies *b);
int clapgpu_characters_update_clock(void *stream, const clapgpu_characters *c, const clapgpu_entities *e, const clapgpu_bodies *b,
                                    const clapgpu_anim_clock *clk, double now, const double *now_dev);

typedef struct clapgpu_move {
    uint32_t        n;
    const uint32_t *body;
    const double   *ray_off;
    const float    *motion;
    const uint8_t  *state;
    const uint8_t  *jump;
    const float    *jump_params;
    float          *velocity;
    float          *normal;
    uint8_t        *airborne;
    uint8_t        *request;
    uint8_t        *applied;
    int32_t        *collision;
    float          *first_frac;
    int32_t        *push_hit;
    uint32_t       *flags;
    const uint32_t *entity;
    const float    *yaw_quat;
} clapgpu_move;
#define CLAPGPU_CS_START      0u
#define CLAPGPU_CS_WAKING     1u
#define CLAPGPU_CS_IDLE       2u
#define CLAPGPU_CS_MOVING     3u
#define CLAPGPU_CS_JUMP_START 4u
#define CLAPGPU_CS_JUMPING    5u
#define CLAPGPU_CS_FALLING    6u
#define CLAPGPU_CS_NONE       0xffu
size_t clapgpu_characters_move_scratch_bytes(uint32_t n_bodies, uint32_t n);
int    clapgpu_characters_move(void *stream, clapgpu_bp *bp, const clapgpu_bodies *b, const clapgpu_world *w,
                               const clapgpu_geoms *statics, const clapgpu_trimesh *meshes,
                               const clapgpu_entities *e ,
                               double dt_sec , const clapgpu_move *m, void *scratch);

size_t clapgpu_characters_order_scratch_bytes(uint32_t n, uint32_t pair_capacity);
int    clapgpu_characters_order(void *stream, clapgpu_bp *order_bp, const clapgpu_bodies *b, const clapgpu_world *w,
                                double dt_sec, const clapgpu_move *m, uint32_t pair_capacity,
                                double *reach , uint32_t *level ,
                                uint32_t *summary , void *scratch);
size_t clapgpu_characters_move_ordered_scratch_bytes(uint32_t n_bodies, uint32_t n, uint32_t pair_capacity);
int    clapgpu_characters_move_ordered(void *stream, clapgpu_bp *bp, clapgpu_bp *order_bp, const clapgpu_bodies *b,
                                       const clapgpu_world *w, const clapgpu_geoms *statics, const clapgpu_trimesh *meshes,
                                       const clapgpu_entities *e, double dt_sec, const clapgpu_move *m, uint32_t pair_capacity,
                                       uint32_t *level , uint32_t *n_levels ,
                                       void *scratch);


#define CLAPGPU_LIGHTS_MAX 128

typedef struct clapgpu_lights {
    uint32_t        nr_lights;
    uint32_t        pad;
    float          *pos;
    const float    *color;
    const float    *attenuation;
    const int32_t  *is_dir;
    const uint32_t *active;
} clapgpu_lights;

void clapgpu_light_grid_dims(uint32_t width, uint32_t height, uint32_t cell, uint32_t *twidth, uint32_t *theight);

int clapgpu_light_grid_compute(void *stream, const clapgpu_lights *lights, const float view_mx[16],
                               const float proj_mx[16], uint32_t width, uint32_t height, uint32_t cell,
                               uint32_t *tiles);

int clapgpu_lights_from_entities(void *stream, const clapgpu_entities *e, uint32_t mode, uint32_t n_carriers,
                                 const uint32_t *carrier_entity, const int32_t *carrier_light,
                                 const float *carrier_off, const clapgpu_lights *lights);


#define CLAPGPU_ANIQ_MAX 4u
#define CLAPGPU_ANI_END_NONE         0u
#define CLAPGPU_ANI_END_IDLE         1u
#define CLAPGPU_ANI_END_START_MOTION 2u
#define CLAPGPU_ANI_END_ANY_TO_JUMP  3u
#define CLAPGPU_ANI_END_HOST         0xffu
#define CLAPGPU_ANI_IDLE           0u
#define CLAPGPU_ANI_START_TO_IDLE  1u
#define CLAPGPU_ANI_MOTION_STOP    2u
#define CLAPGPU_ANI_JUMP_TO_IDLE   3u
#define CLAPGPU_ANI_FALL_TO_IDLE   4u
#define CLAPGPU_ANI_MOTION         5u
#define CLAPGPU_ANI_MOTION_START   6u
#define CLAPGPU_ANI_JUMP_TO_MOTION 7u
#define CLAPGPU_ANI_IDLE_TO_JUMP   8u
#define CLAPGPU_ANI_MOTION_TO_JUMP 9u
#define CLAPGPU_ANI_JUMP           10u
#define CLAPGPU_ANI_FALL           11u
#define CLAPGPU_ANI_NAMES          12u
#define CLAPGPU_ANIQ_ENDED           (1u << 0)
#define CLAPGPU_ANIQ_STARTED         (1u << 1)
#define CLAPGPU_ANIQ_ADVANCED        (1u << 2)
#define CLAPGPU_ANIQ_CB_IDLE         (1u << 3)
#define CLAPGPU_ANIQ_CB_START_MOTION (1u << 4)
#define CLAPGPU_ANIQ_CB_ANY_TO_JUMP  (1u << 5)
#define CLAPGPU_ANIQ_HOST            (1u << 6)
#define CLAPGPU_ANIQ_OVERFLOW        (1u << 7)
#define CLAPGPU_ANIQ_STATE_SHIFT     8u

typedef struct clapgpu_aniq_entry {
    uint16_t animation;
    uint8_t  repeat;
    uint8_t  end;
    float    speed;
} clapgpu_aniq_entry;

typedef struct clapgpu_aniq {
    uint32_t            n;
    uint32_t            n_anims;
    const int32_t      *name_anim;
    const float        *time_end;
    clapgpu_aniq_entry *queue;
    uint8_t            *len;
    int8_t             *cur;
    uint8_t            *cleared;
    double             *ani_time;
    uint8_t            *state;
    uint8_t            *airborne;
    float              *velocity;
    float              *ch_motion;
    const float        *jump_params;
    const int32_t      *mover;
    uint32_t           *pose_anim;
    float              *frame_time;
    uint32_t           *events;
} clapgpu_aniq;

int clapgpu_characters_state(void *stream, const clapgpu_aniq *q, const clapgpu_move *m, double now, const double *now_dev);

int clapgpu_animation_queue_time(void *stream, const clapgpu_aniq *q, double now, const double *now_dev);


typedef struct clapgpu_frame {
    const clapgpu_entities   *entities;
    const uint32_t           *tile_row_start;  uint32_t n_tiles;
    const uint32_t           *level_start;     uint32_t n_levels;
    const clapgpu_frustum    *frustum;
    const clapgpu_bodies     *bodies;
    const clapgpu_world      *world;
    clapgpu_bp               *bp;
    uint32_t *pairs, pair_capacity, *pair_total;
    uint32_t *static_pairs, static_pair_capacity, *static_pair_total;
    const clapgpu_geoms      *body_geoms, *static_geoms;
    clapgpu_contact2 *contacts, *static_contacts;
    uint32_t *contact_total, *static_contact_total;
    uint32_t n_body_links; const uint32_t *link_body, *link_entity;
    const clapgpu_characters *characters;
    const clapgpu_lights     *lights;
    uint32_t n_light_carriers; const uint32_t *carrier_entity; const int32_t *carrier_light; const float *carrier_offset;
    uint32_t light_width, light_height, light_cell; uint32_t *light_tiles;
    const float              *view_mx, *proj_mx;
    const clapgpu_anim_clock *anim_clock;      const double *now_dev;
    const clapgpu_skeleton   *skeleton;
    const clapgpu_animations *animations;
    const clapgpu_pose_batch *pose;
    const clapgpu_skin_batch *skin;
    const clapgpu_particles  *particles;
    uint32_t index_base; uint32_t *visible, *visible_count; void *visible_scratch;
    float cam_pos[3]; const int32_t *force_lod; int32_t *cur_lod, *draw_lod;
    uint32_t flags;
    const clapgpu_trimesh    *meshes;
    clapgpu_contact2 *mesh_contacts; uint32_t *mesh_ref; uint32_t mesh_contact_capacity;
    uint32_t *mesh_contact_total, *mesh_capped;
    uint32_t *mesh_scratch;
    void     *island_scratch;
    uint32_t *island, *island_woken;
    const clapgpu_solver *solver;
    void     *solve_scratch;
    uint32_t  solve_rows_capacity;
    uint32_t *solve_status;
    const clapgpu_move *move;
    double    move_dt_sec;
    void     *move_scratch;
    const clapgpu_aniq *aniq;
} clapgpu_frame;

#define CLAPGPU_FRAME_OVERLAP 1u
#define CLAPGPU_FRAME_PREBIN  2u

int clapgpu_frame_issue(void *stream, const clapgpu_frame *f, double now, uint32_t physics_substeps);

#ifdef __cplusplus
}
#endif
#endif
```

Before: 23.36 billion entity updates/s.

## Emit the ordered visible list inside the tiled entity update kernel

Adds an optional visible-list output to the tiled update kernel. Each tile counts its visible rows, takes an exclusive prefix through a grouped lookback over per-tile and per-group epoch-tagged words, and writes visible indices directly. This is meant to remove the separate compaction launch and its second pass over the visibility mask. The cost is spin-waiting between tiles, extra state memory and a timeout status path. The Python side skips the compaction when the fused list is already valid, but emission is off unless `emit_list` is set.

Result: slower. 22.76 billion entity updates/s (-2.5%).

```diff
diff --git a/clap_amd/_lib.py b/clap_amd/_lib.py
--- a/clap_amd/_lib.py
+++ b/clap_amd/_lib.py
@@ -5,7 +5,7 @@
 _HERE = os.path.dirname(os.path.abspath(__file__))
 LIB_PATH = os.environ.get("CLAPGPU_LIB") or os.path.join(_HERE, "lib", "libclapgpu.so")
 CSRC = os.path.join(_HERE, "csrc")
-ABI_VERSION = 46
+ABI_VERSION = 47
 
 OK = 0
 ERR_NOMEM = -1
@@ -58,6 +58,11 @@
                 ("host_vis_mask", C.c_void_p * EXTRA_VIEWS_MAX)]
 
 
+class VisibleList(C.Structure):
+    _fields_ = [("visible", C.c_void_p), ("count", C.c_void_p), ("index_base", C.c_uint32), ("pad", C.c_uint32),
+                ("state", C.c_void_p)]
+
+
 class Entities(C.Structure):
     _fields_ = [("n", C.c_uint32), ("n_models", C.c_uint32),
                 ("pos_scale", C.c_void_p), ("rot", C.c_void_p), ("parent", C.c_void_p),
@@ -67,7 +72,7 @@
                 ("vis_row_pop", C.c_void_p), ("n_attach", C.c_uint32), ("pad", C.c_uint32),
                 ("attach", C.c_void_p), ("jt_pool", C.c_void_p), ("bind_pool", C.c_void_p),
                 ("attach_local", C.c_void_p), ("bv", C.POINTER(BvQuery)), ("rebuilt_mask", C.c_void_p),
-                ("views", C.POINTER(Views))]
+                ("views", C.POINTER(Views)), ("list", C.POINTER(VisibleList))]
 
 
 class Particles(C.Structure):
@@ -262,7 +267,8 @@
 LIGHTS_MAX = 128
 
 STRUCTS = {
-    "clapgpu_frustum": Frustum, "clapgpu_bv_query": BvQuery, "clapgpu_views": Views, "clapgpu_entities": Entities,
+    "clapgpu_frustum": Frustum, "clapgpu_bv_query": BvQuery, "clapgpu_views": Views, "clapgpu_visible_list": VisibleList,
+    "clapgpu_entities": Entities,
     "clapgpu_particles": Particles, "clapgpu_anim_clock": AnimClock, "clapgpu_skeleton": Skeleton,
     "clapgpu_animations": Animations, "clapgpu_pose_batch": PoseBatch, "clapgpu_skin_batch": SkinBatch,
     "clapgpu_world": World, "clapgpu_bodies": Bodies, "clapgpu_geoms": Geoms, "clapgpu_trimesh_desc": TrimeshDesc,
@@ -298,6 +304,8 @@
                                        C.POINTER(C.c_float), C.c_void_p, C.c_void_p, C.c_void_p]),
     "clapgpu_entities_cull": (C.c_int, [C.c_void_p, C.POINTER(Entities), C.POINTER(Frustum)]),
     "clapgpu_visible_scratch_bytes": (C.c_size_t, [C.c_uint32]),
+    "clapgpu_visible_list_state_bytes": (C.c_size_t, [C.c_uint32]),
+    "clapgpu_visible_list_status": (C.c_int, [C.c_void_p, C.POINTER(VisibleList), C.POINTER(C.c_uint32)]),
     "clapgpu_visible_compact": (C.c_int, [C.c_void_p, C.c_void_p, C.c_void_p, C.c_uint32, C.c_uint32, C.c_void_p,
                                           C.c_void_p, C.c_void_p]),
     "clapgpu_animation_time": (C.c_int, [C.c_void_p, C.POINTER(AnimClock), C.c_double]),
diff --git a/clap_amd/csrc/entities.hip b/clap_amd/csrc/entities.hip
--- a/clap_amd/csrc/entities.hip
+++ b/clap_amd/csrc/entities.hip
@@ -5,6 +5,7 @@
 #include "lm_dev.h"
 #include "entities_row.h"
 #include "entities_args.h"
+#include "entities_list.h"
 
 namespace clapgpu {
 
@@ -12,7 +13,8 @@
 __device__ __forceinline__ void process_row_fast(const EntK &e, const RowIn &in, float4 *tile, const float4 *mt,
                                                  const int lane, const uint32_t row_first, const uint32_t mode,
                                                  const lmd::FrustumK &fr, const int src, const uint32_t parent_seq_now,
-                                                 float (&carry_mx)[16], uint32_t &carry_seq, const XViewsK *xv = nullptr)
+                                                 float (&carry_mx)[16], uint32_t &carry_seq, const XViewsK *xv = nullptr,
+                                                 uint64_t *vis_out = nullptr)
 {
     const uint32_t i = row_first + lane;
     const uint32_t fl = in.fl;
@@ -74,6 +76,7 @@
         const uint64_t m = __ballot(vis);
         e.vis_mask[e0 >> 6] = m;
         e.vis_row_pop[e0 >> 6] = (uint8_t)__popcll(m);
+        if (vis_out) *vis_out = m;
         if constexpr (XV) cull_extra_views(*xv, (fl & CLAPGPU_E_VISIBLE) != 0, fl, bb, (uint32_t)(e0 >> 6), lane);
     }
 }
@@ -145,8 +148,22 @@
     const uint32_t n_rows = (n + WAVE - 1) / WAVE;
     uint32_t row = tile_row_start[t], row_end = tile_row_start[t + 1];
     if (row_end > n_rows) row_end = n_rows;
-    if (row >= row_end)
+    [[maybe_unused]] uint64_t vl_epoch = 0, vl_status = 0, vl_keep = 0, vl_m = 0;
+    [[maybe_unused]] uint32_t vl_row = 0;
+    if constexpr (has_list<XV...>) {
+#if defined(__HIP_DEVICE_COMPILE__)
+        typedef const __attribute__((address_space(4))) uint64_t *ctl_ptr;
+        ctl_ptr ctl = (ctl_ptr)(uintptr_t)list_of(xv...).state;
+#else
+        const uint64_t *ctl = list_of(xv...).state;
+#endif
+        vl_epoch = ctl[VL_EPOCH]; vl_status = ctl[VL_STATUS];
+    }
+    if (row >= row_end) {
+        if constexpr (has_list<XV...>)
+            emit_visible_list(list_of(xv...), e.vis_mask, (uint32_t)vl_epoch, vl_status == 0, 0ull, t, n_tiles, row, row, n, lane);
         return;
+    }
 
     float carry_mx[16];
 #pragma unroll
@@ -182,11 +199,14 @@
             const RowIn nxt = load_row(e, lane, nfirst, ncount);
             frustum_ptr frr = frp;
             asm volatile("" : "+s"(frr));
-            process_row_fast<CULL, sizeof...(XV) != 0>(e, cur, lds_tiles[wave], mt_lds, lane, row_first, mode, *(const lmd::FrustumK *)frr,
-                                                       src, parent_seq_now, carry_mx, carry_seq, xviews_ptr(xv...));
+            process_row_fast<CULL, has_xviews<XV...>>(e, cur, lds_tiles[wave], mt_lds, lane, row_first, mode, *(const lmd::FrustumK *)frr,
+                                                       src, parent_seq_now, carry_mx, carry_seq, xviews_ptr(xv...),
+                                                       has_list<XV...> ? &vl_m : nullptr);
+            if constexpr (has_list<XV...>) { if ((uint32_t)lane == vl_row) vl_keep = vl_m; vl_row++; }
             carry_valid = true;
-            if (!more)
-                return;
+            if (!more) {
+                if constexpr (has_list<XV...>) goto list_tail; else return;
+            }
             have_prev = true;
             cur = nxt;
             row = next;
@@ -202,9 +222,10 @@
         const RowIn nxt = load_row(e, lane, nfirst, ncount);
         frustum_ptr frr = frp;
         asm volatile("" : "+s"(frr));
-        process_row<CULL, true, false, sizeof...(XV) != 0>(e, cur, lds_tiles[wave], lane, row_first, row_count, mode, *(const lmd::FrustumK *)frr,
+        process_row<CULL, true, false, has_xviews<XV...>>(e, cur, lds_tiles[wave], lane, row_first, row_count, mode, *(const lmd::FrustumK *)frr,
                                                            have_prev, row_first - WAVE, carry_mx, carry_seq, carry_valid, nullptr, nullptr,
-                                                           xviews_ptr(xv...));
+                                                           xviews_ptr(xv...), has_list<XV...> ? &vl_m : nullptr);
+        if constexpr (has_list<XV...>) { if ((uint32_t)lane == vl_row) vl_keep = vl_m; vl_row++; }
         if (!more)
             break;
         have_prev = true;
@@ -213,6 +234,12 @@
         row_first = nfirst;
         row_count = ncount;
     }
+[[maybe_unused]] list_tail:
+    if constexpr (has_list<XV...>) {
+        const uint32_t last = tile_row_start[t + 1];
+        emit_visible_list(list_of(xv...), e.vis_mask, (uint32_t)vl_epoch, vl_status == 0, vl_keep, t, n_tiles, tile_row_start[t],
+                          last < n_rows ? last : n_rows, n, lane);
+    }
 }
 
 template <class F> struct first_param;
@@ -221,6 +248,9 @@
               std::is_same<first_param<decltype(&k_entities_tiles<false>)>::type, lmd::FrustumK>::value,
               "k_entities_tiles: the frustum must stay the first kernel argument (it is read at kernarg offset 0)");
 static_assert(std::is_same<first_param<decltype(&k_entities_tiles<true, XViewsK>)>::type, lmd::FrustumK>::value, "... with further views: the same");
+static_assert(std::is_same<first_param<decltype(&k_entities_tiles<true, ListK>)>::type, lmd::FrustumK>::value &&
+              std::is_same<first_param<decltype(&k_entities_tiles<true, XViewsK, ListK>)>::type, lmd::FrustumK>::value,
+              "... and the instantiations that emit the visible list");
 static_assert(alignof(lmd::FrustumK) <= 8, "kernarg offset 0 holds for any alignment the segment start guarantees");
 
 bool make_xviews_k(const clapgpu_entities *e, bool hostio, XViewsK *out)
@@ -327,21 +357,31 @@
 {
     int rc = check_entities(e, frustum != nullptr);
     if (rc) return rc;
-    if (e->n == 0 || n_tiles == 0)
+    const clapgpu_visible_list *list = frustum ? e->list : nullptr;
+    if (e->n == 0 || n_tiles == 0) {
+        if (list)
+            CLAPGPU_HIP(hipMemsetAsync(list->count, 0, sizeof(uint32_t), as_stream(stream)));
         return CLAPGPU_OK;
+    }
     if (!tile_row_start)
         return CLAPGPU_ERR_INVALID_ARGUMENTS;
     const lmd::FrustumK fr = make_frustum_k(frustum);
     const EntK k = to_kernel_args(e);
     XViewsK xv;
     if (!make_xviews_k(e, false, &xv)) return CLAPGPU_ERR_INVALID_ARGUMENTS;
+    ListK lk = {};
+    if (list) { lk.visible = list->visible; lk.count = list->count; lk.state = list->state; lk.index_base = list->index_base; }
     if (k.bv_result)
         CLAPGPU_HIP(hipMemsetAsync(k.bv_result, 0, sizeof(uint64_t), as_stream(stream)));
     rc = prepare_attachments(stream, k);
     if (rc) return rc;
     const uint32_t per_block = ENT_BLOCK / WAVE;
     const dim3 grid((n_tiles + per_block - 1) / per_block), block(ENT_BLOCK);
-    if (frustum && xv.n)
+    if (list && xv.n)
+        hipLaunchKernelGGL((k_entities_tiles<true, XViewsK, ListK>), grid, block, 0, as_stream(stream), fr, k, tile_row_start, n_tiles, e->n, mode, xv, lk);
+    else if (list)
+        hipLaunchKernelGGL((k_entities_tiles<true, ListK>), grid, block, 0, as_stream(stream), fr, k, tile_row_start, n_tiles, e->n, mode, lk);
+    else if (frustum && xv.n)
         hipLaunchKernelGGL((k_entities_tiles<true, XViewsK>), grid, block, 0, as_stream(stream), fr, k, tile_row_start, n_tiles, e->n, mode, xv);
     else if (frustum)
         hipLaunchKernelGGL(k_entities_tiles<true>, grid, block, 0, as_stream(stream), fr, k, tile_row_start, n_tiles,
@@ -350,6 +390,23 @@
         hipLaunchKernelGGL(k_entities_tiles<false>, grid, block, 0, as_stream(stream), fr, k, tile_row_start, n_tiles,
                            e->n, mode);
     CLAPGPU_LAUNCH_CHECK("k_entities_tiles");
+    return CLAPGPU_OK;
+}
+
+extern "C" size_t clapgpu_visible_list_state_bytes(uint32_t n_tiles)
+{
+    const uint32_t n_groups = vl_groups(n_tiles);
+    return (vl_group_words_at(n_tiles) + (size_t)vl_copies(n_groups) * vl_stride(n_groups)) * sizeof(uint64_t);
+}
+
+extern "C" int clapgpu_visible_list_status(void *stream, const clapgpu_visible_list *list, uint32_t *status)
+{
+    if (!list || !list->state || !status)
+        return CLAPGPU_ERR_INVALID_ARGUMENTS;
+    uint64_t word = 0;
+    CLAPGPU_HIP(hipMemcpyAsync(&word, list->state + VL_STATUS, sizeof(word), hipMemcpyDeviceToHost, as_stream(stream)));
+    CLAPGPU_HIP(hipStreamSynchronize(as_stream(stream)));
+    *status = (uint32_t)word;
     return CLAPGPU_OK;
 }
 
diff --git a/clap_amd/csrc/entities_args.h b/clap_amd/csrc/entities_args.h
--- a/clap_amd/csrc/entities_args.h
+++ b/clap_amd/csrc/entities_args.h
@@ -81,6 +81,8 @@
         return CLAPGPU_ERR_INVALID_ARGUMENTS;
     if (need_mask && (!e->vis_mask || !e->vis_row_pop))
         return CLAPGPU_ERR_INVALID_ARGUMENTS;
+    if (e->list && (!e->list->visible || !e->list->count || !e->list->state || (reinterpret_cast<uintptr_t>(e->list->state) & 7u)))
+        return CLAPGPU_ERR_INVALID_ARGUMENTS;
     if (!aligned16(e->pos_scale) || !aligned16(e->rot) || !aligned16(e->model_table) || !aligned16(e->mx) ||
         !aligned16(e->inv_mx) || !aligned16(e->aabb) || !aligned16(e->center))
         return CLAPGPU_ERR_INVALID_ARGUMENTS;
diff --git a/clap_amd/csrc/entities_list.h b/clap_amd/csrc/entities_list.h
--- /dev/null
+++ b/clap_amd/csrc/entities_list.h
@@ -0,0 +1,122 @@
+#pragma once
+#include "common.h"
+#include "entities_row.h"
+#ifdef CLAPGPU_LIST_LOOKBACK
+#include "scan_dev.h"
+#endif
+
+namespace clapgpu {
+
+#if (defined(CLAPGPU_LIST_LOOKBACK) || defined(CLAPGPU_LIST_PAUSE)) && !defined(CLAPGPU_EXPERIMENT)
+#  error "CLAPGPU_LIST_LOOKBACK / CLAPGPU_LIST_PAUSE are experiment switches (profiles/fused_list): add -DCLAPGPU_EXPERIMENT"
+#endif
+#ifndef CLAPGPU_LIST_PAUSE
+#define CLAPGPU_LIST_PAUSE 4
+#endif
+
+constexpr uint64_t VL_VALID = 1ull << 63;
+constexpr uint32_t VL_SPIN_BOUND = 1u << 22;
+
+__device__ __forceinline__ uint64_t vl_word(uint32_t epoch, uint32_t value)
+{
+    return VL_VALID | ((uint64_t)(epoch & 0x7fffffffu) << 32) | value;
+}
+__device__ __forceinline__ bool vl_is(uint64_t w, uint32_t epoch) { return (w >> 32) == (0x80000000u | (epoch & 0x7fffffffu)); }
+__device__ __forceinline__ uint64_t vl_load(const uint64_t *p) { return __hip_atomic_load(p, __ATOMIC_RELAXED, __HIP_MEMORY_SCOPE_AGENT); }
+__device__ __forceinline__ void vl_store(uint64_t *p, uint64_t v) { __hip_atomic_store(p, v, __ATOMIC_RELAXED, __HIP_MEMORY_SCOPE_AGENT); }
+
+__device__ __forceinline__ uint32_t vl_wave_sum(uint32_t v)
+{
+#pragma unroll
+    for (int o = 32; o > 0; o >>= 1) v += __shfl_xor(v, o);
+    return v;
+}
+
+__device__ __forceinline__ void emit_visible_list(const ListK &l, const uint64_t *vis_mask, const uint32_t epoch, bool ok, const uint64_t word0,
+                                                  const uint32_t t, const uint32_t n_tiles, const uint32_t row0, const uint32_t row_end,
+                                                  const uint32_t n, const int lane)
+{
+    const uint32_t n_groups = vl_groups(n_tiles), copies = vl_copies(n_groups), stride = vl_stride(n_groups);
+    uint64_t *ctl = l.state, *tile_w = l.state + VL_CTL_WORDS, *group_w = l.state + vl_group_words_at(n_tiles);
+    const uint32_t nrows = row0 < row_end ? row_end - row0 : 0u;
+
+    uint32_t sum = __popcll(word0);
+    if (nrows > WAVE) {
+        asm volatile("s_waitcnt vmcnt(0)" ::: "memory");
+        for (uint32_t c = WAVE; c < nrows; c += WAVE)
+            sum += c + lane < nrows ? __popcll(vl_load(&vis_mask[row0 + c + lane])) : 0;
+    }
+    sum = vl_wave_sum(sum);
+
+    uint32_t excl = 0;
+#ifdef CLAPGPU_LIST_LOOKBACK
+    if (ok) excl = lb_exclusive(tile_w, t, sum, epoch, reinterpret_cast<uint32_t *>(&ctl[VL_STATUS]), VL_STATUS_TIMEOUT);
+    (void)group_w;
+#else
+    const uint32_t g = t / VL_GROUP, j = t % VL_GROUP;
+    const bool group_last = j == VL_GROUP - 1 || t == n_tiles - 1;
+    const uint64_t *my_groups = group_w + (size_t)(g % copies) * stride;
+    if (ok) {
+        if (lane == 0 && !group_last) vl_store(&tile_w[t], vl_word(epoch, sum));
+        uint32_t in_group = 0, groups = 0, spins = 0;
+        bool published = !group_last;
+        for (uint32_t base = 0; base < g || base == 0; base += WAVE) {
+            bool want_a = base == 0 && (uint32_t)lane < j, want_b = base + lane < g;
+            uint32_t got_a = 0;
+            for (;;) {
+                uint64_t xa = 0, xb = 0;
+                if (want_a) xa = vl_load(&tile_w[g * VL_GROUP + lane]);
+                if (want_b) xb = vl_load(&my_groups[base + lane]);
+                if (want_a && vl_is(xa, epoch)) { got_a = (uint32_t)xa; want_a = false; }
+                if (want_b && vl_is(xb, epoch)) { groups += (uint32_t)xb; want_b = false; }
+                if (base == 0 && __ballot(want_a) == 0ull && !published) {
+                    in_group = vl_wave_sum(got_a);
+                    const uint32_t later = n_groups - 1 - g < copies ? n_groups - 1 - g : copies;
+                    for (uint32_t i = lane; i < later; i += WAVE)
+                        vl_store(&group_w[(size_t)((g + 1 + i) % copies) * stride + g], vl_word(epoch, in_group + sum));
+                    published = true;
+                }
+                if (__ballot(want_a || want_b) == 0ull) break;
+                if (++spins >= VL_SPIN_BOUND) { ok = false; break; }
+                __builtin_amdgcn_s_sleep(CLAPGPU_LIST_PAUSE);
+            }
+            if (base == 0 && !group_last) in_group = vl_wave_sum(got_a);
+            if (!ok) break;
+        }
+        excl = in_group + vl_wave_sum(groups);
+        if (!ok && lane == 0)
+            __hip_atomic_fetch_or(&ctl[VL_STATUS], (uint64_t)VL_STATUS_TIMEOUT, __ATOMIC_RELAXED, __HIP_MEMORY_SCOPE_AGENT);
+    }
+#endif
+
+    uint32_t run = excl;
+    for (uint32_t c = 0; ok && c < nrows; c += WAVE) {
+        const uint64_t word = c == 0 ? word0 : (c + lane < nrows ? vl_load(&vis_mask[row0 + c + lane]) : 0ull);
+        const uint32_t cnt = __popcll(word);
+        const uint32_t incl = wave_prefix_sum(cnt);
+        const uint32_t lo = (uint32_t)word, hi = (uint32_t)(word >> 32), ex = incl - cnt;
+        const uint32_t rows = nrows - c < WAVE ? nrows - c : WAVE;
+        for (uint32_t k = 0; k < rows; k++) {
+            const uint64_t wk = (uint64_t)(uint32_t)__builtin_amdgcn_readfirstlane(__shfl((int)lo, (int)k)) |
+                                ((uint64_t)(uint32_t)__builtin_amdgcn_readfirstlane(__shfl((int)hi, (int)k)) << 32);
+            if (wk == 0) continue;
+            const uint32_t base = run + (uint32_t)__builtin_amdgcn_readfirstlane(__shfl((int)ex, (int)k));
+            if ((wk >> lane) & 1ull) {
+                const uint32_t pos = base + __popcll(wk & ((1ull << lane) - 1ull));
+                if (pos < n)
+                    l.visible[pos] = l.index_base + (row0 + c + k) * 64u + lane;
+            }
+        }
+        run += (uint32_t)__builtin_amdgcn_readfirstlane(__shfl((int)incl, WAVE - 1));
+    }
+
+    if (t == n_tiles - 1 && lane == 0) {
+#ifdef CLAPGPU_LIST_LOOKBACK
+        ok = vl_load(&ctl[VL_STATUS]) == 0;
+#endif
+        __hip_atomic_store(l.count, ok ? excl + sum : 0xFFFFFFFFu, __ATOMIC_RELAXED, __HIP_MEMORY_SCOPE_AGENT);
+        if (ok) vl_store(&ctl[VL_EPOCH], (uint64_t)((epoch + 1u) & 0x7fffffffu));
+    }
+}
+
+}
diff --git a/clap_amd/csrc/entities_row.h b/clap_amd/csrc/entities_row.h
--- a/clap_amd/csrc/entities_row.h
+++ b/clap_amd/csrc/entities_row.h
@@ -1,6 +1,7 @@
 #pragma once
 #include <string.h>
 #include <math.h>
+#include <type_traits>
 #include "common.h"
 #include "lm_dev.h"
 
@@ -41,8 +42,28 @@
     lmd::FrustumK fr[CLAPGPU_EXTRA_VIEWS_MAX];
 };
 
+struct ListK {
+    uint32_t *visible, *count;
+    uint64_t *state;
+    uint32_t  index_base, pad;
+};
+constexpr uint32_t VL_EPOCH = 0, VL_STATUS = 1, VL_CTL_WORDS = 4;
+constexpr uint32_t VL_GROUP = 64;
+constexpr uint32_t VL_STATUS_TIMEOUT = 1u;
+constexpr uint32_t VL_COPIES_MAX = 256;
+__host__ __device__ inline uint32_t vl_groups(uint32_t n_tiles) { return (n_tiles + VL_GROUP - 1) / VL_GROUP; }
+__host__ __device__ inline uint32_t vl_copies(uint32_t n_groups) { return n_groups < VL_COPIES_MAX ? n_groups : VL_COPIES_MAX; }
+__host__ __device__ inline uint32_t vl_stride(uint32_t n_groups) { return (n_groups + 15u) & ~15u; }
+__host__ __device__ inline size_t vl_group_words_at(uint32_t n_tiles) { return ((size_t)VL_CTL_WORDS + n_tiles + 15u) & ~(size_t)15u; }
+
 __device__ __forceinline__ const XViewsK *xviews_ptr() { return nullptr; }
 __device__ __forceinline__ const XViewsK *xviews_ptr(const XViewsK &xv) { return &xv; }
+__device__ __forceinline__ const XViewsK *xviews_ptr(const ListK &) { return nullptr; }
+__device__ __forceinline__ const XViewsK *xviews_ptr(const XViewsK &xv, const ListK &) { return &xv; }
+__device__ __forceinline__ const ListK &list_of(const ListK &l) { return l; }
+__device__ __forceinline__ const ListK &list_of(const XViewsK &, const ListK &l) { return l; }
+template <class... XV> constexpr bool has_xviews = (false || ... || std::is_same<XV, XViewsK>::value);
+template <class... XV> constexpr bool has_list = (false || ... || std::is_same<XV, ListK>::value);
 
 __device__ __forceinline__ bool extra_view_test(const lmd::FrustumK &k, const float (&bb)[6], const float (&lo)[3], const float (&hi)[3],
                                                 const bool box_finite)
@@ -220,7 +241,7 @@
                                             const bool have_prev, const uint32_t prev_first,
                                             float (&carry_mx)[16], uint32_t &carry_seq, bool &carry_valid,
                                             const HostIO *hio = nullptr, const RowPre *pre = nullptr,
-                                            const XViewsK *xv = nullptr)
+                                            const XViewsK *xv = nullptr, uint64_t *vis_out = nullptr)
 {
     const bool in_range = (uint32_t)lane < row_count;
     const uint32_t i = row_first + (in_range ? lane : 0);
@@ -404,6 +425,7 @@
         if (vis && !(fl & CLAPGPU_E_SKIP_CULLING))
             vis = lmd::aabb_in_frustum_fast(fr, bb);
         const uint64_t m = __ballot(vis);
+        if (vis_out) *vis_out = m;
         if (lane == 0) {
             e.vis_mask[e0 >> 6] = m;
             e.vis_row_pop[e0 >> 6] = (uint8_t)__popcll(m);
diff --git a/clap_amd/entities.py b/clap_amd/entities.py
--- a/clap_amd/entities.py
+++ b/clap_amd/entities.py
@@ -75,14 +75,25 @@
             seqs=self.seqs.data_ptr(), mx=self.mx.data_ptr(), inv_mx=self.inv_mx.data_ptr(),
             aabb=self.aabb.data_ptr(), center=self.center.data_ptr(), vis_mask=self.vis_mask.data_ptr(),
             vis_row_pop=self.vis_row_pop.data_ptr())
+        self.emit_list = False
+        self._list_base = 0
+        self._list_valid = False
+        self._list_attached = False
+        if self.tiled:
+            nstate = _lib.lib().clapgpu_visible_list_state_bytes(self.n_tiles)
+            self._list_state = device_array((nstate // 8,), torch.int64, dev)
+            self._list = _lib.VisibleList(visible=self.visible.data_ptr(), count=self.visible_count.data_ptr(),
+                                          index_base=0, state=self._list_state.data_ptr())
 
     def use_vis_buffers(self, vis_mask, vis_row_pop):
+        self._list_valid = False
         self.vis_mask, self.vis_row_pop = vis_mask, vis_row_pop
         self._desc.vis_mask = vis_mask.data_ptr()
         self._desc.vis_row_pop = vis_row_pop.data_ptr()
 
     def set_views(self, frusta):
         dev = self.device
+        self._list_valid = False
         n_rows = (self.n + 63) // 64
         self._views = _lib.Views()
         self._views.n = len(frusta)
@@ -96,6 +107,7 @@
         self._desc.views = C.pointer(self._views) if frusta else None
 
     def compact_view(self, v, index_base=0):
+        self._list_valid = False
         rc = _lib.lib().clapgpu_visible_compact(_stream(), _ptr(self.view_masks[v]), _ptr(self.view_row_pops[v]), self.n,
                                                 index_base, _ptr(self.visible), _ptr(self.visible_count), _ptr(self.scratch))
         _lib.check(rc, "clapgpu_visible_compact")
@@ -135,16 +147,25 @@
     def mq_update(self, frustum=None, all_dirty=False):
         mode = _lib.UPDATE_ALL_DIRTY if all_dirty else 0
         fr = C.byref(frustum) if frustum is not None else None
+        emit = self.emit_list and self.tiled and frustum is not None
+        if emit != self._list_attached:
+            self._desc.list = C.pointer(self._list) if emit else None
+            self._list_attached = emit
+        if emit:
+            self._list.index_base = self._list_base
+        self._list_valid = False
         if self.tiled:
             rc = _lib.lib().clapgpu_entities_update_tiles(_stream(), C.byref(self._desc), _ptr(self.tile_row_start),
                                                           self.n_tiles, mode, fr)
             _lib.check(rc, "clapgpu_entities_update_tiles")
+            self._list_valid = emit
         else:
             rc = _lib.lib().clapgpu_entities_update(_stream(), C.byref(self._desc), self._ls_ptr, self.n_levels,
                                                     mode, fr)
             _lib.check(rc, "clapgpu_entities_update")
 
     def update_level(self, level, frustum=None, all_dirty=False):
+        self._list_valid = False
         first = int(self.level_start[level])
         count = int(self.level_start[level + 1]) - first
         mode = _lib.UPDATE_ALL_DIRTY if all_dirty else 0
@@ -153,10 +174,16 @@
         _lib.check(rc, "clapgpu_entities_update_level")
 
     def cull(self, frustum):
+        self._list_valid = False
         rc = _lib.lib().clapgpu_entities_cull(_stream(), C.byref(self._desc), C.byref(frustum))
         _lib.check(rc, "clapgpu_entities_cull")
 
     def compact_visible(self, index_base=0, two_pass=False):
+        there = self._list_valid and not two_pass and index_base == self._list.index_base
+        self._list_valid = False
+        self._list_base = index_base
+        if there:
+            return
         rc = _lib.lib().clapgpu_visible_compact(_stream(), _ptr(self.vis_mask),
                                                 None if two_pass else _ptr(self.vis_row_pop), self.n, index_base,
                                                 _ptr(self.visible), _ptr(self.visible_count), _ptr(self.scratch))
@@ -180,6 +207,7 @@
 
     def compact_visible_lod(self, cam_pos, force_lod=None, index_base=0):
         self.alloc_lod()
+        self._list_valid = False
         if force_lod is not None:
             self.force_lod = upload(force_lod, np.int32, self.device)
         cp = (C.c_float * 3)(*[float(v) for v in cam_pos])
diff --git a/clap_amd/shard.py b/clap_amd/shard.py
--- a/clap_amd/shard.py
+++ b/clap_amd/shard.py
@@ -75,6 +75,7 @@
         from . import _lib
         self._C, self._lib = C, _lib
         self.batch, self.rank, self.world, self.device = batch, rank, world, device
+        batch.emit_list = False
         self.n_pad = batch.n
         sizes = device_array(world, torch.int64, device)
         sizes[rank] = self.n_pad
diff --git a/include/clapgpu.h b/include/clapgpu.h
--- a/include/clapgpu.h
+++ b/include/clapgpu.h
@@ -27,7 +27,7 @@
 int clapgpu_init(int device);
 const char *clapgpu_last_error(void);
 void clapgpu_test_fail_after(int launches);
-#define CLAPGPU_ABI_VERSION 46u
+#define CLAPGPU_ABI_VERSION 47u
 uint32_t clapgpu_abi_version(void);
 
 int clapgpu_malloc(void **dev, size_t bytes);
@@ -75,6 +75,16 @@
     uint8_t        *vis_row_pop[CLAPGPU_EXTRA_VIEWS_MAX];
     uint64_t       *host_vis_mask[CLAPGPU_EXTRA_VIEWS_MAX];
 } clapgpu_views;
+
+typedef struct clapgpu_visible_list {
+    uint32_t *visible;
+    uint32_t *count;
+    uint32_t  index_base;
+    uint32_t  pad;
+    uint64_t *state;
+} clapgpu_visible_list;
+size_t clapgpu_visible_list_state_bytes(uint32_t n_tiles);
+int clapgpu_visible_list_status(void *stream, const clapgpu_visible_list *list, uint32_t *status);
 
 typedef struct clapgpu_entities {
     uint32_t        n;
@@ -101,6 +111,7 @@
     const clapgpu_bv_query *bv;
     uint64_t       *rebuilt_mask;
     const clapgpu_views *views;
+    const clapgpu_visible_list *list;
 } clapgpu_entities;
 
 #define CLAPGPU_UPDATE_ALL_DIRTY  (1u << 0)
```
